# dakom/awsm-renderer

Hardware: AMD Instinct MI355X
Metric: frames/sec + shaded Mpix/s, 4K Sponza glTF, 1/2/4/8 MI355X (higher is better)
Workload: dtype f32; 1 GPU; Sponza-class procedural atrium (configs[3]): 262144 triangles, 25 materials, 69 textures, 3840x2160, geometry pass + opaque pass, single-sample, MipmapMode::None; triangles=262144, width=3840, height=2160, draws=92, frame_overlap=True, stream_handoff=device flags (k_handoff_signal / k_handoff_wait), camera=orbit, one turn per 240 frames, environment=uniform cubes (builder default), opaque_route=lean (k_shade_lean + k_shade_todo), library=awsm-renderer_amd/libawsm_hip.so

## Files before the change

### awsm-renderer_amd/csrc/awsm_hip.cpp

```cpp
#include <hip/hip_runtime.h>
#include <algorithm>
#include <cmath>
#include <cstdarg>
#include <cstdio>
#include <cstdlib>
#include <cstring>
#include <ctime>
#include <string>
#include <vector>

#include "ctx.hpp"
#include "launch.hpp"

using namespace awsm;

namespace {

constexpr int kLeanWgsPerCu = 0;

inline FrameBufs* pass_slots(AwsmHipCtx* c, PassKind kind) {
    FrameBufs* const sets[kPassKinds] = {c->fb, c->tr, c->hud, c->htr, c->shadow};
    return sets[kind];
}
inline FrameBufs& pass_bufs(AwsmHipCtx* c, PassKind kind) { return pass_slots(c, kind)[c->slot]; }
// ... 153 lines not shown
    return AWSM_OK;
}

uint32_t mip_levels_full(uint32_t w, uint32_t h) {
    uint32_t m = std::max(w, h), n = 0;
    while (m > 1u) { m >>= 1; n++; }
    return n + 1u;
}

}

namespace {

void shard(const AwsmHipCtx* c, uint32_t* y0, uint32_t* y1) {
    *y0 = c->y0; *y1 = c->y1;
    if (*y1 == 0 || *y1 > c->height) *y1 = c->height;
    if (*y0 > *y1) *y0 = *y1;
}

void log_dirty(AwsmHipCtx* c, AwsmBuf which, size_t lo, size_t hi) {
    if (c->geometry_cache) c->dirty_log.log((uint32_t)which, lo, hi, c->write_seq);
}

int sync_scene(AwsmHipCtx* c) {
    if (!c->scene_dirty) return AWSM_OK;
    c->write_seq++;
    { int rcb = scene_write_barrier(c, false); if (rcb) return rcb; }
    for (int i = 0; i < AWSM_BUF_COUNT; i++) c->scene.buf[i] = (const uint8_t*)c->bufs[i].ptr;
    c->scene.lut_rg16f = (const uint16_t*)c->lut.ptr;
    int rc = upload_small(c, c->scene_dev, &c->scene, sizeof(DevScene));
    if (rc) return rc;
    c->scene_dirty = false;
    c->scene_uploads++;
    return AWSM_OK;
}

void bind_pass(FrameDev& f, const FrameBufs& b) {
    f.bin_capacity = b.bin_capacity;
    f.draws = (const DrawDev*)b.draws_dev.ptr;
    f.clip = (float4*)b.clip.ptr; f.nrm = (float4*)b.nrm.ptr; f.tan = (float4*)b.tan.ptr;
    f.tri_info = (uint32_t*)b.tri_flags.ptr;
    f.tri_rec = (TriRec*)b.tri_rec.ptr;
    f.tile_count = (uint32_t*)b.tile_count.ptr; f.tile_offset = (uint32_t*)b.tile_offset.ptr;
    f.tile_cursor = (uint32_t*)b.tile_cursor.ptr; f.bin_list = (uint32_t*)b.bin_list.ptr;
    f.tile_order = (uint32_t*)b.tile_order.ptr;
    f.scan_tmp = (uint32_t*)b.scan_tmp.ptr;
    f.tile_split = (uint32_t*)b.tile_split.ptr; f.raster_scratch = (unsigned long long*)b.raster_scratch.ptr;
    f.raster_extra_cap = b.raster_extra_cap; f.raster_slot_cap = b.raster_slot_cap;
    f.big_list = (uint32_t*)b.big_list.ptr;
    f.counters = (uint32_t*)b.counters.ptr;
    f.vis = (unsigned long long*)b.vis.ptr;
}

struct FrameView { bool hud_keys, merged; };
inline FrameView world_view() { return {false, false}; }
inline FrameView frame_view(const AwsmHipCtx* c) { return {c->hud_geometry_done, c->hud_merged}; }

void fill_frame(AwsmHipCtx* c, FrameDev* f, FrameView view) {
    memset(f, 0, sizeof *f);
    const PassList& world = c->lists[kPassWorld];
    const PassList& hud = c->lists[kPassHud];
    uint32_t y0, y1;
    shard(c, &y0, &y1);
    f->width = c->width; f->height = c->height; f->y0 = y0; f->y1 = y1; f->sy0 = y0; f->sy1 = y1;
    if (c->msaa && (y0 > 0 || y1 < c->height)) {
        f->y0 = y0 > 0 ? y0 - 1 : 0; f->y1 = std::min(c->height, y1 + 1);
    }
    f->tiles_x = (c->width + kTile - 1) / kTile;
    f->band_n = 1; f->band_r = 0; f->out_compact = 0;
    f->tile_row0 = f->y0 >> kTileShift;
    f->tiles_y = (f->y1 > f->y0) ? ((f->y1 + kTile - 1) / kTile - f->tile_row0) : 0;
    if (c->band_n > 1) {
        const uint32_t rows_full = (c->height + kTile - 1) / kTile;
        f->band_n = c->band_n; f->band_r = c->band_r; f->out_compact = c->band_compact;
        f->tile_row0 = c->band_r;
        f->tiles_y = c->band_r < rows_full ? (rows_full - c->band_r + c->band_n - 1) / c->band_n : 0;
    }
    f->n_draws = (uint32_t)world.draws.size();
    f->total_tris = world.total_tris; f->total_verts = 3u * world.total_tris;
    bind_pass(*f, FB(c));
    f->draw_shade = (DrawShadeDev*)FB(c).draw_shade.ptr;
    f->tex_slots = (TexSlotDev*)FB(c).tex_slots.ptr;
    f->draw_mat = (DrawMatDev*)FB(c).draw_mat.ptr;
    const bool lean_ok = !(c->flags & AWSM_CFG_GENERAL_SHADE_ONLY) && (uint64_t)c->width * c->height * (c->msaa == 4 ? 32u : 8u) < (1ull << 32) && (c->msaa == 0 || (c->msaa_edge_bits[c->slot].ptr && c->msaa_cells[c->slot].ptr)) && FB(c).tri_shade.ptr && FB(c).draw_lean.ptr && c->shade_todo[c->slot].ptr && ((uint64_t)world.total_tris + (view.merged ? hud.total_tris : 0u)) * kTriRecBytes < (1ull << 32) &&
                         c->bufs[AWSM_BUF_ATTR_DATA].size < (1ull << 32) - 64;
    f->tri_shade = lean_ok ? (uint4*)FB(c).tri_shade.ptr : nullptr;
    f->attr_data_bytes = (uint32_t)std::min<size_t>(c->bufs[AWSM_BUF_ATTR_DATA].size, 0xFFFFFFFFu);
    f->draw_lean = lean_ok ? (LeanDrawDev*)FB(c).draw_lean.ptr : nullptr;
    f->shade_todo = (uint32_t*)c->shade_todo[c->slot].ptr;
    f->shade_todo_cap = f->shade_todo ? (uint32_t)(c->shade_todo[c->slot].size / 4 - 4 - 1024) : 0u;
    f->lean_next = f->shade_todo ? f->shade_todo + 4 + f->shade_todo_cap : nullptr;
    f->lean_grid = c->lean_grid;
#ifdef AWSM_STAMP
    {
        static unsigned long long* stamps = nullptr;
        if (!stamps && hipMalloc((void**)&stamps, 4ull * 16384 * 8 * 8) == hipSuccess) (void)hipMemset(stamps, 0, 4ull * 16384 * 8 * 8);
        f->stamps = stamps;
        static bool told = false;
        if (!told) { told = true; FILE* fp = fopen("/tmp/awsm_stamps_ptr", "w"); if (fp) { fprintf(fp, "%llu\n", (unsigned long long)(uintptr_t)stamps); fclose(fp); } }
    }
#endif
    f->poison = c->handoff_poison ? c->handoff_poison + c->slot : nullptr;
    f->host_bin_status = c->counters_host + 16 + 2 * c->slot;
    f->frame_serial = c->frame_serial;
    f->camera = (const uint8_t*)FB(c).camera.ptr;
    f->camera_snap = nullptr; f->camera_snap_words = 0;
    memcpy(f->pix2view, FB(c).pix2view, sizeof f->pix2view); memcpy(f->view_rot, FB(c).view_rot, sizeof f->view_rot); memcpy(f->cam_pos, FB(c).cam_pos, sizeof f->cam_pos);
    memcpy(f->ortho_view_dir, FB(c).ortho_view_dir, sizeof f->ortho_view_dir); f->cam_ortho = FB(c).cam_ortho;
    f->msaa = c->msaa;
    f->msaa_color0 = (float4*)c->msaa_color0[c->slot].ptr;
    f->msaa_edges = (uint32_t*)c->msaa_edges[c->slot].ptr;
    f->msaa_edge_bits = (lean_ok && c->msaa == 4) ? (unsigned long long*)c->msaa_edge_bits[c->slot].ptr : nullptr;
    f->msaa_cells = (uint2*)c->msaa_cells[c->slot].ptr;
    f->hud_vis = view.hud_keys ? (const unsigned long long*)c->hud[c->slot].vis.ptr : nullptr;
    f->hud_draws = (const DrawDev*)c->hud[c->slot].draws_dev.ptr; f->hud_tri_info = (const uint32_t*)c->hud[c->slot].tri_flags.ptr;
    if (view.hud_keys && view.merged) {
        f->n_draws = (uint32_t)c->hud_combined.size();
        f->total_tris = world.total_tris + hud.total_tris; f->total_verts = 3u * f->total_tris;
        f->vis = (unsigned long long*)c->merged_vis[c->slot].ptr;
        f->hud_draws = f->draws; f->hud_tri_info = f->tri_info;
    }
    f->hud_pass = 0;
    f->msaa_halo = (const unsigned long long*)c->msaa_halo;
    f->halo_bands = c->band_n > 1 ? ((c->height + kTile - 1) / kTile + c->band_n - 1) / c->band_n : 0u;
    f->out_rgba16f = (uint16_t*)(c->bound_out ? (uint8_t*)c->bound_out - (size_t)c->out_first_row * c->width * 8 : c->out16[c->slot].ptr);
    f->out_rgba32f = (float*)c->out32[c->slot].ptr;
    f->lights_pre = (float4*)c->lights_pre[c->slot].ptr;
    f->lights_cap = (uint32_t)(c->lights_pre[c->slot].size / 32);
}

void compose_pixel_to_view(AwsmHipCtx* c, FrameBufs& b) {
    float cam[128];
    memcpy(cam, c->camera_host, 512);
    const float* proj = cam + 16; const float* inv_proj = cam + 64; const float* inv_view = cam + 80;
    const double W = (double)c->width, H = (double)c->height;
    const double A[16] = {2.0 / W, 0, 0, 0,   0, -2.0 / H, 0, 0,   0, 0, 1, 0,   1.0 / W - 1.0, 1.0 - 1.0 / H, 0, 1};
    for (int col = 0; col < 4; col++) for (int row = 0; row < 4; row++) {
        double s = 0.0;
        for (int k = 0; k < 4; k++) s += (double)inv_proj[k * 4 + row] * A[col * 4 + k];
        b.pix2view[col * 4 + row] = (float)s;
    }
    for (int col = 0; col < 3; col++) for (int row = 0; row < 3; row++) b.view_rot[col * 3 + row] = inv_view[col * 4 + row];
    for (int i = 0; i < 3; i++) b.cam_pos[i] = cam[96 + i];
    b.cam_ortho = proj[15] > 0.9f ? 1u : 0u;
    const double vx = inv_view[8], vy = inv_view[9], vz = inv_view[10], l = std::sqrt(vx * vx + vy * vy + vz * vz);
    b.ortho_view_dir[0] = l > 0.0 ? (float)(vx / l) : 0.0f; b.ortho_view_dir[1] = l > 0.0 ? (float)(vy / l) : 0.0f; b.ortho_view_dir[2] = l > 0.0 ? (float)(vz / l) : 1.0f;
}

int record(AwsmHipCtx* c, int which, hipStream_t s = nullptr) {
    if (!c->stage_timers) { c->ev_valid[which] = false; return AWSM_OK; }
    HIPCHK(c, hipEventRecord(c->ev[which], s ? s : c->stream));
    c->ev_valid[which] = true;
    return AWSM_OK;
}

AwsmHipCtx::ResolveKey resolve_key(AwsmHipCtx* c, const FrameDev& f) {
    AwsmHipCtx::ResolveKey k;
    memset(&k, 0, sizeof k);
    k.write_seq = c->write_seq + (c->scene_dirty ? 1u : 0u); k.draws_version = FB(c).draws_version;
    k.ptrs[0] = f.draw_shade; k.ptrs[1] = f.draw_mat; k.ptrs[2] = f.tex_slots; k.ptrs[3] = f.draw_lean; k.ptrs[4] = f.lights_pre;
    k.n_draws = f.n_draws; k.mipmap = c->last_opaque.mipmap; k.has_opaque = c->last_opaque.has_opaque; k.lights_cap = f.lights_cap;
    return k;
}
bool resolve_stale(AwsmHipCtx* c, const FrameDev& f) {
    const AwsmHipCtx::ResolveKey k = resolve_key(c, f);
    return memcmp(&k, &c->resolved[c->slot], sizeof k) != 0;
}

void fill_geometry_cache(AwsmHipCtx* c, FrameDev* f, bool replay) {
    FrameBufs& b = FB(c);
    f->wcache = (float4*)b.wcache.ptr;
    f->cache_on = 0; f->prev_draws = nullptr; f->prev_n_draws = 0; f->n_dirty = 0; f->cache_serial = b.cache_serial;
    if (!c->geometry_cache || replay || !b.cache_valid || !b.wcache.ptr || b.cache_had_tri_shade != (f->tri_shade != nullptr)) return;
    std::vector<DirtyRange> r;
    if (!c->dirty_log.ranges_since(b.cache_seq, kMaxDirtyRanges, r)) return;
    for (size_t i = 0; i < r.size(); i++) { f->dirty[i][0] = r[i].buf; f->dirty[i][1] = r[i].lo; f->dirty[i][2] = r[i].hi; }
    f->n_dirty = (uint32_t)r.size();
    f->prev_draws = (const DrawDev*)(b.cached_is_prev ? b.draws_prev.ptr : b.draws_dev.ptr);
    f->prev_n_draws = b.cached_n_draws;
    f->cache_on = f->prev_draws ? 1u : 0u;
}


inline void enqueue_binning(const FrameDev& f, bool has_tris, hipStream_t s) {
    if (has_tris) { awsm_launch_bin_count(&f, s); awsm_launch_bin_big(&f, 0, s); }
    awsm_launch_bin_scan(&f, s);
    if (has_tris) { awsm_launch_bin_fill(&f, s); awsm_launch_bin_big(&f, 1, s); }
}
int clear_empty_pass(AwsmHipCtx* c, const FrameBufs& b, uint32_t n_tiles, hipStream_t s) {
    HIPCHK(c, hipMemsetAsync(b.counters.ptr, 0, kCtrWords * sizeof(uint32_t), s));
    HIPCHK(c, hipMemsetAsync((uint32_t*)b.counters.ptr + 12, 0, 2 * sizeof(uint32_t), s));
    if (n_tiles) HIPCHK(c, hipMemsetAsync(b.tile_count.ptr, 0, n_tiles * sizeof(uint32_t), s));
    return AWSM_OK;
}

int enqueue_geometry(AwsmHipCtx* c, bool replay = false) {
    HostTrace ht(c->frame_serial);
    const PassList& world = c->lists[kPassWorld];
    FrameDev f;
    fill_frame(c, &f, world_view());
    fill_geometry_cache(c, &f, replay);
    f.block_draw = FB(c).block_map_valid ? (const uint32_t*)FB(c).block_map.ptr : nullptr;
    f.cache_mark = (c->stage_timers && FB(c).cache_mark.size >= (size_t)world.n_blocks * 4) ? (uint32_t*)FB(c).cache_mark.ptr : nullptr;
    const uint32_t n_tiles = f.tiles_x * f.tiles_y;
    int rc = sync_scene(c);
    if (rc) return rc;
    ht.mark("geometry: sync_scene");
    if (c->overlap && c->shade_pending[c->slot]) { HIPCHK(c, wait_slot_free(c)); c->shade_pending[c->slot] = false; }
    if (c->bufs[AWSM_BUF_CAMERA].ptr && !replay) {
        const size_t cam_bytes = std::min<size_t>(512, c->bufs[AWSM_BUF_CAMERA].size);
        if (world.total_tris && n_tiles) { f.camera_snap = (uint32_t*)FB(c).camera.ptr; f.camera_snap_words = (uint32_t)(cam_bytes / 4); }
        else HIPCHK(c, hipMemcpyAsync(FB(c).camera.ptr, c->bufs[AWSM_BUF_CAMERA].ptr, cam_bytes, hipMemcpyDeviceToDevice, c->stream));
    }
    if (c->overlap) {
        c->uploads_recorded[c->slot] = false;
        if (resolve_stale(c, f)) { HIPCHK(c, hipEventRecord(c->ev_uploads[c->slot], c->stream)); c->uploads_recorded[c->slot] = true; }
        c->geom_write_seq[c->slot] = c->write_seq;
    }
    ht.mark("geometry: slot wait + upload event");
    const bool has_geometry = world.total_tris && n_tiles;
    if (!has_geometry && (rc = clear_empty_pass(c, FB(c), n_tiles, c->stream))) return rc;
    if (c->trace_dev) awsm_launch_handoff_signal(nullptr, 0u, trace_slot(c, 0), c->stream);
    if ((rc = record(c, EV_START))) return rc;
#ifdef AWSM_DEBUG_SWITCHES
    static const int knockout_env = getenv("AWSM_DEBUG_KNOCKOUT") ? atoi(getenv("AWSM_DEBUG_KNOCKOUT")) : 0;
    const int knockout = c->frame_serial > 8 ? knockout_env : 0;
#else
    const int knockout = 0;
#endif
    if (has_geometry && !(knockout & 1)) awsm_launch_transform(c->scene_dev, &f, world.n_blocks, c->stream);
    if ((rc = record(c, EV_TRANSFORM))) return rc;
    ht.mark("geometry: transform launch");
    if (n_tiles && !(knockout & 2)) enqueue_binning(f, world.total_tris != 0, c->stream);
    if ((rc = record(c, EV_BIN))) return rc;
    ht.mark("geometry: bin launches");
    if (n_tiles && !(knockout & 4)) awsm_launch_raster(&f, c->stream);
    if ((rc = record(c, EV_RASTER))) return rc;
    ht.mark("geometry: raster launch");
    HIPCHK(c, hipGetLastError());
    {
        FrameBufs& b = FB(c);
        b.cache_valid = has_geometry && !(knockout & 1) && b.wcache.ptr != nullptr;
        b.cached_n_draws = (uint32_t)world.draws.size(); b.cached_is_prev = false;
// ... 402 lines not shown
    if (hipGetDeviceProperties(&prop, c->device) != hipSuccess) return bail(AWSM_ERR_DEVICE);
    if (strncmp(prop.gcnArchName, "gfx950", 6) != 0) {
        fprintf(stderr, "awsm_hip: device %d is %s; this library carries gfx950 code objects only\n", c->device, prop.gcnArchName);
        return bail(AWSM_ERR_NO_DEVICE);
    }
    if (cfg->stream) { c->stream = (hipStream_t)cfg->stream; c->own_stream = false; }
    else { if (hipStreamCreateWithFlags(&c->stream, hipStreamNonBlocking) != hipSuccess) return bail(AWSM_ERR_DEVICE); c->own_stream = true; }
    for (int i = 0; i < EV_COUNT; i++) if (hipEventCreate(&c->ev[i]) != hipSuccess) return bail(AWSM_ERR_DEVICE);
    if (hipMalloc((void**)&c->scene_dev, sizeof(DevScene)) != hipSuccess) return bail(AWSM_ERR_OUT_OF_MEMORY);
    c->overlap = (cfg->flags & AWSM_CFG_OVERLAP_FRAMES) != 0;
    { const char* e = getenv("AWSM_GEOMETRY_CACHE"); c->geometry_cache = !(e && e[0] == '0'); }
    {
        const char* e = getenv("AWSM_LEAN_WGS_PER_CU");
        const int per_cu = e ? atoi(e) : (c->overlap ? kLeanWgsPerCu : 0);
        c->lean_grid = per_cu > 0 ? (uint32_t)(per_cu * prop.multiProcessorCount) & ~7u : 0u;
    }
    for (int s = 0; s < n_slots(c); s++) {
        for (PassKind k : {kPassWorld, kPassTransparent, kPassHudTransparent, kPassHud}) {
            DevBuf& ctr = pass_slots(c, k)[s].counters;
            if (hipMalloc(&ctr.ptr, 16 * sizeof(uint32_t)) != hipSuccess || (k == kPassWorld && hipMemset(ctr.ptr, 0, 16 * sizeof(uint32_t)) != hipSuccess)) return bail(AWSM_ERR_OUT_OF_MEMORY);
            ctr.size = 16 * sizeof(uint32_t);
        }
        if (hipMalloc(&c->fb[s].camera.ptr, 512) != hipSuccess || hipMemset(c->fb[s].camera.ptr, 0, 512) != hipSuccess) return bail(AWSM_ERR_OUT_OF_MEMORY);
        c->fb[s].camera.size = 512;
    }

    if (c->overlap) {
        for (int s = 0; s < kSlots; s++) {
#ifdef AWSM_DEBUG_SWITCHES
            if (const char* m = getenv("AWSM_SHADE_CU_MASK")) {
                std::vector<uint32_t> words;
                for (const char* p = m; *p; ) { char* end = nullptr; words.push_back((uint32_t)strtoul(p, &end, 16)); p = (*end == ',') ? end + 1 : end; if (end == p && *p) break; }
                if (words.empty() || hipExtStreamCreateWithCUMask(&c->shade_streams[s], (uint32_t)words.size(), words.data()) != hipSuccess) return bail(AWSM_ERR_DEVICE);
            } else
#endif
            if (hipStreamCreateWithFlags(&c->shade_streams[s], hipStreamNonBlocking) != hipSuccess) return bail(AWSM_ERR_DEVICE);
            const unsigned ev_flags = hipEventDisableTiming | hipEventReleaseToDevice;
            if (hipEventCreateWithFlags(&c->ev_geom_done[s], ev_flags) != hipSuccess || hipEventCreateWithFlags(&c->ev_shade_done[s], ev_flags) != hipSuccess ||
                hipEventCreateWithFlags(&c->ev_uploads[s], ev_flags) != hipSuccess) return bail(AWSM_ERR_DEVICE);
            if (s == 0 && hipEventCreateWithFlags(&c->ev_flush, hipEventDisableTiming) != hipSuccess) return bail(AWSM_ERR_DEVICE);
        }
    }
    if (hipHostMalloc((void**)&c->counters_host, (16 + 2 * kSlots + 1) * sizeof(uint32_t), hipHostMallocDefault) != hipSuccess) return bail(AWSM_ERR_OUT_OF_MEMORY);
    memset(c->counters_host, 0, (16 + 2 * kSlots + 1) * sizeof(uint32_t));
    if (c->overlap) {
        const char* e = getenv("AWSM_DEVICE_HANDOFF");
        c->handoff = !(e && e[0] == '0');
        { int khz = 0; if (hipDeviceGetAttribute(&khz, hipDeviceAttributeWallClockRate, c->device) == hipSuccess && khz > 0) c->clock_khz = (uint32_t)khz; }
        double budget_ms = 4000.0;
        if (const char* p = getenv("AWSM_HANDOFF_TIMEOUT_MS")) { const double v = atof(p); if (v > 0.0) budget_ms = v; }
        c->handoff_budget_ticks = (unsigned long long)(budget_ms * (double)c->clock_khz) + 1ull;
        if (hipMalloc((void**)&c->handoff_flags, 3 * kSlots * sizeof(uint32_t)) != hipSuccess || hipMalloc((void**)&c->handoff_poison, kSlots * sizeof(uint32_t)) != hipSuccess) return bail(AWSM_ERR_OUT_OF_MEMORY);
        if (hipMemset(c->handoff_flags, 0, 3 * kSlots * sizeof(uint32_t)) != hipSuccess || hipMemset(c->handoff_poison, 0xFF, kSlots * sizeof(uint32_t)) != hipSuccess ||
            hipDeviceSynchronize() != hipSuccess) return bail(AWSM_ERR_DEVICE);
        if (const char* d = getenv("AWSM_TEST_HANDOFF_DROP")) c->handoff_test_drop = (uint32_t)atoi(d);
        for (int k = 0; c->handoff && k < 2 * kSlots; k++) {
            hipStream_t ss = c->shade_streams[k % kSlots], waiter = k < kSlots ? ss : c->stream, setter = k < kSlots ? c->stream : ss;
            const uint32_t serial = ++c->geom_sig[0];
            awsm_launch_handoff_wait(c->handoff_flags, serial, 10ull * c->clock_khz , handoff_timeouts(c), 0u, nullptr, 0u, waiter);
            awsm_launch_handoff_signal(c->handoff_flags, serial, nullptr, setter);
            if (hipStreamSynchronize(waiter) != hipSuccess || hipStreamSynchronize(setter) != hipSuccess) return bail(AWSM_ERR_DEVICE);
            if (*(volatile uint32_t*)handoff_timeouts(c) != 0u) { c->handoff = false; c->handoff_timeouts_seen = *(volatile uint32_t*)handoff_timeouts(c); }
        }
    }
    memset(&c->scene, 0, sizeof c->scene);
    c->scene.skybox_rgba[3] = 1.0f;
    for (int i = 0; i < 3; i++) { c->scene.prefiltered_rgb[i] = 1.0f; c->scene.irradiance_rgb[i] = 1.0f; }
    *out = c;
    return AWSM_OK;
}

int awsm_hip_destroy(AwsmHipCtx* c) {
    if (!c) return AWSM_ERR_INVALID_ARGUMENT;
    (void)hipSetDevice(c->device);
    if (c->stream) (void)hipStreamSynchronize(c->stream);
    (void)sync_shade_streams(c);
    auto fr = [](DevBuf& b) { if (b.ptr) (void)hipFree(b.ptr); b.ptr = nullptr; b.size = 0; };
    for (auto& b : c->bufs) fr(b);
    for (auto& b : c->tex) fr(b);
    for (auto& b : c->tex_kinds) fr(b);
    for (auto& b : c->merged_vis) fr(b);
    fr(c->pose_records);
    fr(c->env_stage); fr(c->env_tables); fr(c->env_rows); fr(c->env_filter_tab); if (c->ev_env_copy) (void)hipEventDestroy(c->ev_env_copy);
    fr(c->lut); for (auto& b : c->cube_tex) fr(b); for (auto& b : c->cube_bordered) fr(b); fr(c->digest); for (auto& b : c->shade_todo) fr(b); for (int sl = 0; sl < kSlots; sl++) { fr(c->msaa_color0[sl]); fr(c->msaa_edges[sl]); fr(c->msaa_edge_bits[sl]); fr(c->msaa_cells[sl]); } fr(c->mip_kinds); for (auto& b : c->out16) fr(b); for (auto& b : c->out32) fr(b); fr(c->comp16); fr(c->comp32); fr(c->grid_layer); for (auto& b : c->lights_pre) fr(b);
    for (auto& b : c->ssao_layers) fr(b);
    for (auto& b : c->taa_img) fr(b); fr(c->taa_layers);
    for (auto& b : c->sel_tables) fr(b);
    fr(c->sel_layers);
    for (auto& b : c->shadow_layers) fr(b); for (auto& b : c->shadow_cam) fr(b); for (DevScene* sc : c->shadow_scene) if (sc) (void)hipFree(sc);
    for (auto& b : c->display8) fr(b); fr(c->effects16); fr(c->bloom_a); fr(c->bloom_b); fr(c->dof_lc); fr(c->dof_blur);
    for (int k = 0; k < kPassKinds * kSlots; k++) {
        FrameBufs& b = pass_slots(c, (PassKind)(k / kSlots))[k % kSlots];
        fr(b.vis); fr(b.wpos); fr(b.frag_rec); fr(b.frag_color); fr(b.frag_first); fr(b.tex_slots); fr(b.draw_mat); fr(b.clip); fr(b.nrm); fr(b.tan); fr(b.tri_rec); fr(b.tri_flags); fr(b.tri_shade); fr(b.draw_lean); fr(b.draws_dev); fr(b.draw_shade); fr(b.tile_count); fr(b.tile_offset);
        fr(b.wcache); fr(b.draws_prev); fr(b.cache_mark); fr(b.block_map); fr(b.tile_cursor); fr(b.tile_order); fr(b.scan_tmp); fr(b.tile_split); fr(b.raster_scratch); fr(b.bin_list); fr(b.big_list); fr(b.counters); fr(b.camera);
    }
    for (hipStream_t st : c->shade_streams) if (st) (void)hipStreamDestroy(st);
    for (int i = 0; i < kSlots; i++) { if (c->ev_geom_done[i]) (void)hipEventDestroy(c->ev_geom_done[i]); if (c->ev_shade_done[i]) (void)hipEventDestroy(c->ev_shade_done[i]); if (c->ev_uploads[i]) (void)hipEventDestroy(c->ev_uploads[i]); }
    if (c->ev_flush) (void)hipEventDestroy(c->ev_flush);
    if (c->scene_dev) (void)hipFree(c->scene_dev);
    if (c->stage) (void)hipHostFree(c->stage);
    if (c->counters_host) (void)hipHostFree(c->counters_host);
    if (c->handoff_flags) (void)hipFree(c->handoff_flags);
    if (c->handoff_poison) (void)hipFree(c->handoff_poison);
    if (c->trace_dev) (void)hipFree(c->trace_dev);
    for (int i = 0; i < EV_COUNT; i++) if (c->ev[i]) (void)hipEventDestroy(c->ev[i]);
    if (c->own_stream && c->stream) (void)hipStreamDestroy(c->stream);
    delete c;
    return AWSM_OK;
}

int awsm_hip_device_info(AwsmHipCtx* c, char* name_out, size_t name_cap, uint32_t* cu_count, uint64_t* hbm_bytes) {
    if (!c) return AWSM_ERR_INVALID_ARGUMENT;
    hipDeviceProp_t prop;
    HIPCHK(c, hipGetDeviceProperties(&prop, c->device));
    if (name_out && name_cap) snprintf(name_out, name_cap, "%s (%s)", prop.name, prop.gcnArchName);
    if (cu_count) *cu_count = (uint32_t)prop.multiProcessorCount;
    if (hbm_bytes) *hbm_bytes = (uint64_t)prop.totalGlobalMem;
    return AWSM_OK;
}

int awsm_hip_buffer_create(AwsmHipCtx* c, AwsmBuf which, size_t bytes) {
    if (!c || (int)which < 0 || which >= AWSM_BUF_COUNT) return fail(c, AWSM_ERR_INVALID_ARGUMENT, "buffer_create: bad buffer id %d", (int)which);
    HIPCHK(c, hipSetDevice(c->device));
    { int rcb = scene_write_barrier(c); if (rcb) return rcb; }
    log_dirty(c, which, 0, ~size_t(0));
    if (bytes && c->bufs[which].ptr && c->bufs[which].size == bytes) {
        if (which == AWSM_BUF_CAMERA) memset(c->camera_host, 0, sizeof c->camera_host);
        HIPCHK(c, hipMemsetAsync(c->bufs[which].ptr, 0, bytes + 16, c->stream));
        return AWSM_OK;
    }
    int rc = dev_realloc(c, c->bufs[which], bytes ? bytes + 16 : 0, true);
    if (rc) return rc;
    if (bytes) c->bufs[which].size = bytes;
    if (which == AWSM_BUF_CAMERA) memset(c->camera_host, 0, sizeof c->camera_host);
    if (which == AWSM_BUF_LIGHTS) for (int sl = 0; sl < n_slots(c); sl++) if ((rc = dev_realloc(c, c->lights_pre[sl], std::max<size_t>(bytes / 64, 1) * 32, true))) return rc;
    c->scene_dirty = true;
    return AWSM_OK;
}

int awsm_hip_buffer_write(AwsmHipCtx* c, AwsmBuf which, size_t dst_off, const void* src, size_t len) {
    if (!c || (int)which < 0 || which >= AWSM_BUF_COUNT || (!src && len)) return fail(c, AWSM_ERR_INVALID_ARGUMENT, "buffer_write: bad argument");
    if ((dst_off & 3) || (len & 3)) return fail(c, AWSM_ERR_INVALID_ARGUMENT, "buffer_write: offset %zu / size %zu not 4-byte aligned", dst_off, len);
    DevBuf& b = c->bufs[which];
    if (!b.ptr) return fail(c, AWSM_ERR_NOT_READY, "buffer_write: buffer %d was never created", (int)which);
    if (dst_off > b.size || len > b.size - dst_off) return fail(c, AWSM_ERR_OUT_OF_RANGE, "buffer_write: [%zu,+%zu) outside buffer %d of %zu bytes", dst_off, len, (int)which, b.size);
    if (len == 0) return AWSM_OK;
    HIPCHK(c, hipSetDevice(c->device));
    if (which != AWSM_BUF_CAMERA) { int rcb = scene_write_barrier(c); if (rcb) return rcb; log_dirty(c, which, dst_off, dst_off + len); }
    else { if (dst_off < 512) memcpy(c->camera_host + dst_off, src, std::min<size_t>(len, 512 - dst_off)); c->camera_written_since_snapshot = true; }
    uint8_t* dst = (uint8_t*)b.ptr + dst_off;
    if (len <= (1u << 20)) return upload_small(c, dst, src, len);
    HIPCHK(c, hipMemcpyAsync(dst, src, len, hipMemcpyHostToDevice, c->stream));
    HIPCHK(c, hipStreamSynchronize(c->stream));
    return AWSM_OK;
}

int awsm_hip_skin_pose_records_write(AwsmHipCtx* c, uint32_t first, uint32_t n, const AwsmSkinPoseRecord* records) {
    if (!c || (!records && n)) return fail(c, AWSM_ERR_INVALID_ARGUMENT, "skin_pose_records_write: bad argument");
    static_assert(sizeof(AwsmSkinPoseRecord) == 72, "k_skin_pose reads 72-byte records");
    std::vector<AwsmSkinPoseRecord>& host = c->pose_records_host;
    if (first > host.size() || n > 0x03000000u - first) return fail(c, AWSM_ERR_OUT_OF_RANGE, "skin_pose_records_write: [%u,+%u) with %zu records resident", first, n, host.size());
    if (n == 0) return AWSM_OK;
    for (uint32_t i = 0; i < n; i++)
        if ((records[i].transform_offset & 3u) || (records[i].matrix_offset & 3u)) return fail(c, AWSM_ERR_INVALID_ARGUMENT, "skin_pose_records_write: record %u has an offset that is not a multiple of 4", first + i);
    HIPCHK(c, hipSetDevice(c->device));
    { int rcb = scene_write_barrier(c, false); if (rcb) return rcb; }
    std::vector<AwsmSkinPoseRecord> next(host.begin(), host.end());
// ... 6 lines not shown
        if (rc) { host.clear(); return rc; }
        lo = 0; count = next.size();
    }
    constexpr size_t kChunk = 8192;
    for (size_t at = lo; at < lo + count; at += kChunk) {
        const size_t m = std::min(kChunk, lo + count - at);
        int rc = upload_small(c, (uint8_t*)c->pose_records.ptr + at * sizeof(AwsmSkinPoseRecord), next.data() + at, m * sizeof(AwsmSkinPoseRecord));
        if (rc) { host.clear(); return rc; }
    }
    host.swap(next);
    return AWSM_OK;
}

int awsm_hip_skin_pose(AwsmHipCtx* c, const uint32_t* ids, uint32_t n) {
    if (!c || (!ids && n)) return fail(c, AWSM_ERR_INVALID_ARGUMENT, "skin_pose: bad argument");
    if (n == 0) return AWSM_OK;
    const DevBuf& tb = c->bufs[AWSM_BUF_TRANSFORMS];
    const DevBuf& mb = c->bufs[AWSM_BUF_SKIN_MATRICES];
    if (!tb.ptr || !mb.ptr) return fail(c, AWSM_ERR_NOT_READY, "skin_pose: the transforms or the skin matrices buffer was never created");
    const std::vector<AwsmSkinPoseRecord>& host = c->pose_records_host;
    std::vector<uint32_t> offs(n);
    for (uint32_t i = 0; i < n; i++) {
        if (ids[i] >= host.size()) return fail(c, AWSM_ERR_OUT_OF_RANGE, "skin_pose: record id %u (list entry %u) with %zu records resident", ids[i], i, host.size());
        const AwsmSkinPoseRecord& r = host[ids[i]];
        if (tb.size < 64 || r.transform_offset > tb.size - 64) return fail(c, AWSM_ERR_OUT_OF_RANGE, "skin_pose: record %u reads [%u,+64) of a transforms buffer of %zu bytes", ids[i], r.transform_offset, tb.size);
        if (mb.size < 64 || r.matrix_offset > mb.size - 64) return fail(c, AWSM_ERR_OUT_OF_RANGE, "skin_pose: record %u writes [%u,+64) of a skin matrices buffer of %zu bytes", ids[i], r.matrix_offset, mb.size);
        offs[i] = r.matrix_offset;
    }
    HIPCHK(c, hipSetDevice(c->device));
    { int rcb = scene_write_barrier(c); if (rcb) return rcb; }
    std::sort(offs.begin(), offs.end());
    for (size_t i = 0; i < offs.size();) {
        size_t j = i + 1;
        while (j < offs.size() && offs[j] <= offs[j - 1] + 64u) j++;
        log_dirty(c, AWSM_BUF_SKIN_MATRICES, offs[i], (size_t)offs[j - 1] + 64);
        i = j;
    }
    constexpr uint32_t kChunk = 65536;
    for (uint32_t at = 0; at < n; at += kChunk) {
        const uint32_t m = std::min(kChunk, n - at);
        uint8_t* st;
        int rc = stage_alloc(c, (size_t)m * 4, &st);
        if (rc) return rc;
        memcpy(st, ids + at, (size_t)m * 4);
        awsm_launch_skin_pose(c->pose_records.ptr, (const uint32_t*)st, m, tb.ptr, mb.ptr, c->stream);
        HIPCHK(c, hipGetLastError());
    }
    return AWSM_OK;
}

int awsm_hip_buffer_read(AwsmHipCtx* c, AwsmBuf which, size_t offset, void* dst, size_t len) {
    if (!c || (int)which < 0 || which >= AWSM_BUF_COUNT || (!dst && len)) return fail(c, AWSM_ERR_INVALID_ARGUMENT, "buffer_read: bad argument");
    const DevBuf& b = c->bufs[which];
    if (!b.ptr) return fail(c, AWSM_ERR_NOT_READY, "buffer_read: buffer %d was never created", (int)which);
    if (offset > b.size || len > b.size - offset) return fail(c, AWSM_ERR_OUT_OF_RANGE, "buffer_read: [%zu,+%zu) outside buffer %d of %zu bytes", offset, len, (int)which, b.size);
    if (len == 0) return AWSM_OK;
    HIPCHK(c, hipSetDevice(c->device));
    HIPCHK(c, hipStreamSynchronize(c->stream));
    HIPCHK(c, hipMemcpy(dst, (const uint8_t*)b.ptr + offset, len, hipMemcpyDeviceToHost));
    return AWSM_OK;
}

int awsm_hip_resize(AwsmHipCtx* c, uint32_t width, uint32_t height, uint32_t msaa) {
    if (!c || width == 0 || height == 0 || width > 16384 || height > 16384) return fail(c, AWSM_ERR_INVALID_ARGUMENT, "resize: bad size %ux%u", width, height);
    if (msaa == 1) msaa = 0;
    if (msaa != 0 && msaa != 4) return fail(c, AWSM_ERR_UNSUPPORTED, "resize: MSAA x%u (the reference supports None or 4, anti_alias.rs:28-38)", msaa);
    HIPCHK(c, hipSetDevice(c->device));
    const size_t px = (size_t)width * height, samples = msaa == 4 ? 4 : 1;
    int rc;
    if ((rc = sync_all(c))) return rc;
    for (int s = 0; s < n_slots(c); s++) {
        if ((rc = dev_realloc(c, c->fb[s].vis, px * samples * 8, false))) return rc;
        HIPCHK(c, hipMemsetAsync(c->fb[s].vis.ptr, 0xFF, px * samples * 8, c->stream));
    }
    if (msaa == 4) for (int sl = 0; sl < n_slots(c); sl++) {
        const size_t blocks = (size_t)((width + 15) / 16) * ((height + 15) / 16);
        if ((rc = dev_realloc(c, c->msaa_edge_bits[sl], blocks * 4 * 16, true))) return rc;
        if ((rc = dev_realloc(c, c->msaa_cells[sl], px * 8, false))) return rc;
        if ((rc = dev_realloc(c, c->msaa_color0[sl], px * 16, false))) return rc;
        if ((rc = dev_realloc(c, c->msaa_edges[sl], blocks * 260, false))) return rc;
    }
    c->msaa = msaa;
    for (int sl = 0; sl < n_slots(c); sl++) if ((rc = dev_realloc(c, c->shade_todo[sl], ((size_t)((width + 15) / 16) * ((height + 15) / 16) * 4 + 4 + 1024) * 4, true))) return rc;
    for (int sl = 0; sl < n_slots(c); sl++) {
        if ((rc = dev_realloc(c, c->out16[sl], px * 8, true))) return rc;
        if ((c->flags & AWSM_CFG_PARITY_TAP) && (rc = dev_realloc(c, c->out32[sl], px * 16, true))) return rc;
    }
    c->width = width; c->height = height;
    c->y0 = c->y1 = 0;
    c->band_n = 1; c->band_r = 0; c->band_compact = 0;
    c->geometry_done = c->opaque_done = c->transparent_done = c->hud_transparent_done = c->post_done = false;
    c->last_display = nullptr;
    c->taa_have = false; c->taa_serial = 0; c->taa_resolved = false;
    return AWSM_OK;
}

int awsm_hip_set_shard_bands(AwsmHipCtx* c, uint32_t n, uint32_t r, uint32_t compact_output) {
    if (!c) return AWSM_ERR_INVALID_ARGUMENT;
    if (c->width == 0) return fail(c, AWSM_ERR_NOT_READY, "set_shard_bands before resize");
    if (n == 0 || r >= n) return fail(c, AWSM_ERR_INVALID_ARGUMENT, "set_shard_bands: need r < n (got n=%u r=%u)", n, r);
    { int rcs = sync_all(c); if (rcs) return rcs; }
    c->y0 = c->y1 = 0;
    c->band_n = n; c->band_r = n > 1 ? r : 0; c->band_compact = (n > 1 && compact_output) ? 1u : 0u;
    return AWSM_OK;
}

uint32_t awsm_hip_msaa_halo_bands(AwsmHipCtx* c) {
    return (c && c->band_n > 1 && c->height) ? ((c->height + kTile - 1) / kTile + c->band_n - 1) / c->band_n : 0u;
}

int awsm_hip_msaa_halo_export(AwsmHipCtx* c, void* dst, size_t bytes) {
    if (!c || !dst) return AWSM_ERR_INVALID_ARGUMENT;
    if (c->msaa != 4 || c->band_n <= 1) return fail(c, AWSM_ERR_INVALID_ARGUMENT, "msaa_halo_export: only for MSAA x4 with band sharding");
    if (!c->geometry_done) return fail(c, AWSM_ERR_NOT_READY, "msaa_halo_export before geometry_pass");
    const uint32_t bands = awsm_hip_msaa_halo_bands(c);
    if (bytes < (size_t)bands * 2 * c->width * 8) return fail(c, AWSM_ERR_INVALID_ARGUMENT, "msaa_halo_export: %zu bytes, %zu needed (%u bands x 2 rows x %u keys)", bytes, (size_t)bands * 2 * c->width * 8, bands, c->width);
    HIPCHK(c, hipSetDevice(c->device));
    FrameDev f;
    fill_frame(c, &f, frame_view(c));
    awsm_launch_msaa_halo_export(&f, (unsigned long long*)dst, bands, c->stream);
    HIPCHK(c, hipGetLastError());
    return AWSM_OK;
}

int awsm_hip_msaa_halo_bind(AwsmHipCtx* c, const void* gathered, size_t bytes) {
    if (!c) return AWSM_ERR_INVALID_ARGUMENT;
    if (gathered && bytes == 0) return fail(c, AWSM_ERR_INVALID_ARGUMENT, "msaa_halo_bind: zero-sized array");
    c->msaa_halo = gathered; c->msaa_halo_bytes = bytes;
    return AWSM_OK;
}

int awsm_hip_set_shard_rows(AwsmHipCtx* c, uint32_t y0, uint32_t y1) {
    if (!c) return AWSM_ERR_INVALID_ARGUMENT;
    if (c->width == 0) return fail(c, AWSM_ERR_NOT_READY, "set_shard_rows before resize");
    { int rcs = sync_all(c); if (rcs) return rcs; }
    c->band_n = 1; c->band_r = 0; c->band_compact = 0;
    if (y0 == 0 && y1 == 0) { c->y0 = c->y1 = 0; return AWSM_OK; }
    if (y0 >= y1 || y1 > c->height) return fail(c, AWSM_ERR_INVALID_ARGUMENT, "set_shard_rows: need y0 < y1 <= height (got %u,%u)", y0, y1);

    c->y0 = y0; c->y1 = y1;
    return AWSM_OK;
}

int awsm_hip_geometry_pass(AwsmHipCtx* c, const AwsmDraw* draws, uint32_t n) {
    if (!c || (!draws && n)) return AWSM_ERR_INVALID_ARGUMENT;
    if (c->width == 0) return fail(c, AWSM_ERR_NOT_READY, "geometry_pass before resize");
    static const AwsmBuf need[] = {AWSM_BUF_TRANSFORMS, AWSM_BUF_CAMERA, AWSM_BUF_GEOM_META, AWSM_BUF_VIS_GEOM_DATA};
    if (n) for (AwsmBuf b : need) if (!c->bufs[b].ptr) return fail(c, AWSM_ERR_NOT_READY, "geometry_pass: buffer %d missing", (int)b);
    HIPCHK(c, hipSetDevice(c->device));

    HostTrace ht(c->frame_serial + 1u);
    std::vector<DrawDev> new_draws;
    uint64_t tris = 0, blocks = 0;
    int rc = build_draw_list(c, "geometry_pass", draws, n, AWSM_BUF_VIS_GEOM_DATA, 168u, new_draws, &tris, &blocks);
    if (rc) return rc;
    ht.mark("geometry_pass: draw list");
    if ((rc = handoff_check(c))) return rc;
    c->hud_geometry_done = false; c->hud_merged = false;
    c->frame_serial++;
    if (c->overlap) {
        c->slot = (c->slot + 1) % kSlots;
        if (c->shade_pending[c->slot]) {
            if (hipEventQuery(c->ev_shade_done[c->slot]) != hipSuccess) HIPCHK(c, wait_slot_free(c));
            c->shade_pending[c->slot] = false;
        }
    }
// ... 953 lines not shown
```

### awsm-renderer_amd/csrc/ctx.hpp

```cpp
#pragma once
#include <hip/hip_runtime.h>
#include <stddef.h>
#include <stdint.h>
#include <string>
#include <vector>

#include "frame_params.hpp"
#include "dirty_log.hpp"

namespace awsm {

#ifndef AWSM_SLOTS
#define AWSM_SLOTS 2
#endif
constexpr int kSlots = AWSM_SLOTS;
struct DevBuf {
    void* ptr = nullptr;
    size_t size = 0;
};

enum { EV_START = 0, EV_TRANSFORM, EV_BIN, EV_RASTER, EV_SHADE_BEGIN, EV_SHADE_LEAN, EV_SHADE, EV_FWD_BEGIN, EV_FWD, EV_COUNT };

enum PassKind : uint8_t { kPassWorld = 0, kPassTransparent, kPassHud, kPassHudTransparent, kPassShadow };
constexpr int kPassKinds = 5;
// ... 12 lines not shown
    DevBuf tri_shade, draw_lean;
    DevBuf clip, nrm, tan, tri_rec, tri_flags, draws_dev, draw_shade, tile_count, tile_offset, tile_cursor, tile_order, bin_list, big_list, counters, vis;
    DevBuf camera;
    DevBuf scan_tmp;
    DevBuf tile_split, raster_scratch;
    uint32_t raster_extra_cap = 0, raster_slot_cap = 0;
    uint32_t bin_capacity = 0;
    float pix2view[16] = {}, view_rot[9] = {}, cam_pos[3] = {}, ortho_view_dir[3] = {};
    uint32_t cam_ortho = 0;
    size_t tri_cap = 0, draw_cap = 0;
    uint32_t sized_w = 0, sized_h = 0;
    std::vector<DrawDev> draws_uploaded;
    void* draws_uploaded_ptr = nullptr;
    bool draws_uploaded_valid = false;
    uint64_t draws_version = 0;
    std::vector<DrawDev> tail_uploaded;
    void* tail_uploaded_ptr = nullptr;
    size_t tail_uploaded_at = 0;
    bool tail_uploaded_valid = false;
    DevBuf wcache, draws_prev;
    DevBuf block_map;
    bool block_map_valid = false;
    DevBuf cache_mark;
    uint32_t cached_n_draws = 0;
    bool cache_valid = false;
    bool cached_is_prev = false;
    bool cache_had_tri_shade = false;
    uint64_t cache_seq = 0;
    uint32_t cache_serial = 0;
    PassKind kind = kPassWorld;
    uint8_t slot = 0;
};

}

using namespace awsm;

struct AwsmHipCtx {
    int device = 0;
    uint32_t flags = 0;
    hipStream_t stream = nullptr;
    bool own_stream = false;
    bool stage_timers = true;
    std::string last_error;

    DevBuf bufs[AWSM_BUF_COUNT];
    bool camera_written_since_snapshot = false;
    uint8_t camera_host[512] = {};
    DevScene scene{};
    DevScene* scene_dev = nullptr;
    bool scene_dirty = true;
    DevBuf tex[kMaxTexArrays];
    DevBuf lut;
    DevBuf cube_tex[3], cube_bordered[3];
    DevBuf env_stage, env_tables, env_rows, env_filter_tab;
    hipEvent_t ev_env_copy = nullptr;
    DevBuf tex_kinds[kMaxTexArrays];
    uint32_t tex_srgb[64] = {};
    bool tex_srgb_made = false;

    DevBuf pose_records;
    std::vector<AwsmSkinPoseRecord> pose_records_host;

    uint32_t width = 0, height = 0;
    uint32_t y0 = 0, y1 = 0;
    uint32_t band_n = 1, band_r = 0, band_compact = 0;
    uint32_t msaa = 0;
    DevBuf mip_kinds;
    DevBuf msaa_color0[kSlots], msaa_edges[kSlots];
    DevBuf msaa_edge_bits[kSlots];
    DevBuf msaa_cells[kSlots];
    DevBuf out16[kSlots], out32[kSlots];
    DevBuf digest;
    uint32_t lean_grid = 0;
    DevBuf shade_todo[kSlots];
    void* bound_out = nullptr;
    size_t bound_out_bytes = 0;
    const uint8_t* slot_out_lo[kSlots] = {}; const uint8_t* slot_out_hi[kSlots] = {};

    bool overlap = false;
    hipStream_t shade_streams[kSlots] = {};
    bool shade_recorded[kSlots] = {};
    bool uploads_recorded[kSlots] = {};
    struct ResolveKey { uint64_t write_seq, draws_version; const void* ptrs[5]; uint32_t n_draws, mipmap, has_opaque, lights_cap; } resolved[kSlots] = {};
    hipEvent_t ev_geom_done[kSlots] = {}, ev_shade_done[kSlots] = {}, ev_uploads[kSlots] = {} ;
    hipEvent_t ev_flush = nullptr;
    uint64_t write_seq = 0, geom_write_seq[kSlots] = {};
    DirtyLog dirty_log;
    bool geometry_cache = true;
    uint32_t cache_blocks_last = 0;
    bool shade_pending[kSlots] = {};
    bool handoff = false;
    uint32_t* handoff_flags = nullptr;
    uint32_t geom_sig[kSlots] = {}, shade_sig[kSlots] = {}, lean_sig[kSlots] = {};
    bool lean_flagged[kSlots] = {};
    unsigned long long handoff_budget_ticks = 400000000ull;
    uint32_t clock_khz = 100000;
    uint32_t* handoff_poison = nullptr;
    uint32_t handoff_timeouts_seen = 0;
    uint32_t handoff_dropped_frames = 0;
    bool handoff_error_pending = false;
    uint32_t handoff_test_drop = 0;
    FrameBufs fb[kSlots];
    FrameBufs tr[kSlots];
    FrameBufs hud[kSlots];
    bool hud_geometry_done = false;
    bool hud_merged = false;
    DevBuf merged_vis[kSlots];
    std::vector<DrawDev> hud_combined;
    bool transparent_done = false, hud_transparent_done = false;
    FrameBufs htr[kSlots];
    struct GridState { bool on = false; float p[20] = {}; } grid, grid_pass[kSlots];
    DevBuf grid_layer;
    struct SelectionState {
        bool on = false;
        uint32_t flags = 0, radius = 0;
        float outline_color[4] = {}, box_color[4] = {}, half_width = 0, hidden_alpha = 0, depth_epsilon = 0;
        std::vector<uint32_t> keys;
        std::vector<float> boxes;
    } sel, sel_pass[kSlots];
    DevBuf sel_tables[kSlots], sel_layers;
    DevBuf comp16, comp32;
    DevBuf display8[kSlots], effects16, bloom_a, bloom_b, dof_lc, dof_blur;
    void* bound_display = nullptr;
    size_t bound_display_bytes = 0;
    void* last_display = nullptr;
    bool post_done = false;
    AwsmPostParams post_params{};
    DevBuf lights_pre[kSlots];
    void* bound_comp = nullptr;
    size_t bound_comp_bytes = 0;
    const void* msaa_halo = nullptr;
    size_t msaa_halo_bytes = 0;
    const void* opaque_src = nullptr;
    size_t opaque_src_bytes = 0;
    int slot = 0;
    PassList lists[kPassKinds];
    std::vector<AwsmDraw> draws_api;
    bool geometry_done = false, opaque_done = false;
    AwsmOpaqueParams last_opaque{};
    uint32_t overflow_retries = 0;
    bool has_opaque_for_stats() const { return !opaque_done || last_opaque.has_opaque != 0; }

    uint8_t* stage = nullptr;
    size_t stage_cap = 0, stage_head = 0;
    uint32_t* counters_host = nullptr;
    uint32_t frame_serial = 0, status_seen[kSlots] = {};
    uint32_t dropped_frames = 0;
    uint32_t out_first_row = 0;
    bool out_rows_mode = false;

    hipEvent_t ev[EV_COUNT] = {};
    bool ev_valid[EV_COUNT] = {};

    unsigned long long* trace_dev = nullptr;
    uint32_t trace_cap = 0;

    struct SsaoState { bool on = false; float p[4] = {}; } ssao, ssao_pass[kSlots];
    DevBuf ssao_layers[kSlots];
    size_t ssao_px[kSlots] = {};

    FrameBufs shadow[kSlots];
    DevScene* shadow_scene[kSlots] = {};
    uint64_t shadow_scene_seq[kSlots] = {}, scene_uploads = 0;
    DevBuf shadow_cam[kSlots];
    bool shadow_done = false;
    struct ShadowState { bool on = false; AwsmShadow p{}; float light_view_proj[16] = {}; } shadow_pass[kSlots];
    DevBuf shadow_layers[kSlots];
    size_t shadow_px[kSlots] = {};

    struct TaaState {
        bool on = false;
        float feedback = 0.1f;
        uint32_t flags = 0;
        float jitter[2] = {};
        float reproject[16] = {1, 0, 0, 0, 0, 1, 0, 0, 0, 0, 1, 0, 0, 0, 0, 1};
    } taa, taa_pass;
    DevBuf taa_img[2], taa_layers;
    int taa_cur = 0;
    bool taa_have = false;
    bool taa_frame_hist = false;
    uint32_t taa_serial = 0;
    bool taa_resolved = false;
    TaaArgs taa_args{};
};

#define HIPCHK(c, call)                                                                            \
    do {                                                                                           \
        hipError_t e_ = (call);                                                                    \
        if (e_ != hipSuccess)                                                                      \
            return fail((c), e_ == hipErrorOutOfMemory ? AWSM_ERR_OUT_OF_MEMORY : AWSM_ERR_DEVICE, \
                        "%s failed: %s (%s:%d)", #call, hipGetErrorString(e_), __FILE__, __LINE__); \
    } while (0)

#define AWSM_HIDDEN __attribute__((visibility("hidden")))

namespace awsm {

AWSM_HIDDEN int fail(AwsmHipCtx* c, int code, const char* fmt, ...);
AWSM_HIDDEN hipError_t sync_shade_streams(AwsmHipCtx* c);
AWSM_HIDDEN int dev_realloc(AwsmHipCtx* c, DevBuf& b, size_t bytes, bool zero);
AWSM_HIDDEN int dev_reserve(AwsmHipCtx* c, DevBuf& b, size_t bytes);
AWSM_HIDDEN int stage_alloc(AwsmHipCtx* c, size_t len, uint8_t** out);
AWSM_HIDDEN int upload_small(AwsmHipCtx* c, void* dst, const void* src, size_t len);
AWSM_HIDDEN int scene_write_barrier(AwsmHipCtx* c, bool is_write = true);
AWSM_HIDDEN int sync_all(AwsmHipCtx* c);
AWSM_HIDDEN uint32_t mip_levels_full(uint32_t w, uint32_t h);

}
```

### awsm-renderer_amd/csrc/frame_params.hpp

```cpp
#pragma once
#include <hip/hip_runtime.h>
#include <stdint.h>
#include "../../include/awsm_hip.h"

namespace awsm {

constexpr int kTile = 32;
constexpr int kTileShift = 5;
constexpr int kMaxTexArrays = 64;
constexpr int kMaxSamplers = 32;

constexpr uint32_t kDrawInstanced = 0x80u;

struct DrawDev {
    uint32_t geom_meta_off;
    uint32_t vis_data_off;
    uint32_t tri_count;
    uint32_t flags;
    uint32_t first_tri;
    uint32_t first_block;
    uint32_t inst_off;
    uint32_t pad1;
};

struct DrawShadeDev {
    uint32_t first_tri;
    uint32_t material_word;
    uint32_t attr_indices_word;
    uint32_t attr_data_word;
    uint32_t stride_words;
    uint32_t uv_sets_index;
    uint32_t flags;
    uint32_t color_sets;
};

struct TexSlotDev {
    const uint32_t* base;
    uint32_t width, height;
    uint32_t flags;
    float tt[6];
    uint32_t layer_levels;
    const uint32_t* level_off;
    const uint32_t* array_base;
};
static_assert(sizeof(TexSlotDev) == 64, "TexSlotDev must be 64 bytes");
constexpr int kCoreTextures = 5;

struct DrawMatDev {
    float base_color[4];
    float metallic, roughness, normal_scale, occlusion_strength;
    float emissive[3];
    float ior;
    uint32_t shader_alpha;
    uint32_t debug_bitmask;
    uint32_t ext_mask;
    float alpha_cutoff;
};
static_assert(sizeof(DrawMatDev) == 64, "DrawMatDev must be 64 bytes");

struct LeanDrawDev {
    uint32_t flags;
    float metallic, roughness, normal_scale;
    float base_color[3]; float occlusion_strength;
    float emissive[3];
    float normal_bias;
    uint32_t tex[kCoreTextures][2];
    float occlusion_bias;
    uint32_t pad1;
    uint32_t gtex[kCoreTextures][4];
    float tt[6];
    uint32_t pad2[2];
};
static_assert(sizeof(LeanDrawDev) == 208, "LeanDrawDev must be 208 bytes");

constexpr int kMaxMipLevels = 16;
struct TexArrayDev {
    const uint8_t* texels;
    uint32_t width, height, layers;
    uint32_t mips;
    uint32_t level_off[kMaxMipLevels];
};

struct CubeDev {
    const uint2* texels;
    uint32_t size, mips;
    uint32_t level_off[kMaxMipLevels];
    const uint2* bordered;
    uint32_t b_level_off[kMaxMipLevels];
};
enum { kCubeSkybox = 0, kCubePrefiltered = 1, kCubeIrradiance = 2 };

struct DevScene {
    const uint8_t* buf[AWSM_BUF_COUNT];
    TexArrayDev tex[kMaxTexArrays];
    AwsmSampler samplers[kMaxSamplers];
    uint32_t n_tex, n_samplers;
    float skybox_rgba[4];
    float prefiltered_rgb[4];
    float irradiance_rgb[4];
    const uint16_t* lut_rg16f;
    uint32_t lut_w, lut_h;
    CubeDev cube[3];
};

struct TriRec;
constexpr size_t kTriRecBytes = 80;
constexpr uint32_t kMaxDirtyRanges = 12;

enum CounterWord : uint32_t { kCtrBinned = 0, kCtrEntries, kCtrOverflow, kCtrCovered, kCtrBig, kCtrFragments, kCtrFragOverflow, kCtrExtraItems, kCtrWords };

struct FrameDev {
    uint32_t width, height;
    uint32_t y0, y1;
    uint32_t sy0, sy1;
    uint32_t tiles_x, tiles_y;
    uint32_t tile_row0;
    uint32_t band_n, band_r;
    uint32_t out_compact;
    uint32_t n_draws;
    uint32_t total_tris;
    uint32_t total_verts;
    uint32_t rank0, block0;
    uint32_t bin_capacity;
    uint32_t has_opaque;
    uint32_t mipmap;
    uint32_t aniso;
    uint32_t msaa;
    const uint8_t* camera;
    float pix2view[16];
    float view_rot[9];
    float cam_pos[3];
    float ortho_view_dir[3];
    uint32_t cam_ortho;
    const DrawDev* draws;
    DrawShadeDev* draw_shade;
    TexSlotDev* tex_slots;
    DrawMatDev* draw_mat;
    float4* lights_pre;
    uint32_t lights_cap;
    float4* clip;
    float4* nrm;
    float4* tan;
    float4* wpos;
    const uint32_t* block_draw;
    float4* wcache;
    const DrawDev* prev_draws;
    uint32_t prev_n_draws;
    uint32_t cache_on;
    uint32_t cache_serial;
    uint32_t* cache_mark;
    uint32_t n_dirty;
    uint32_t dirty[12][3];
    TriRec* tri_rec;
    uint32_t* tri_info;
    uint4* tri_shade;
    uint32_t attr_data_bytes;
    LeanDrawDev* draw_lean;
    uint32_t* shade_todo;
    uint32_t shade_todo_cap;
    uint32_t* lean_done_flag;
    uint32_t lean_done_serial;
    uint32_t* camera_snap;
    uint32_t camera_snap_words;
    uint32_t* lean_next;
    uint32_t lean_grid;
    uint32_t* tile_count;
    uint32_t* tile_offset;
    uint32_t* tile_cursor;
    uint32_t* scan_tmp;
    uint32_t* tile_order;
    uint32_t* tile_split;
    unsigned long long* raster_scratch;
    uint32_t raster_extra_cap, raster_slot_cap;
    uint32_t* bin_list;
    uint32_t* big_list;
#ifdef AWSM_STAMP
    unsigned long long* stamps;
#endif
    const uint32_t* poison;
    uint32_t* host_bin_status;
    uint32_t frame_serial;
    uint32_t* counters;
    unsigned long long* vis;
    uint16_t* out_rgba16f;
    float* out_rgba32f;
    float4* msaa_color0;
    uint32_t* msaa_edges;
    unsigned long long* msaa_edge_bits;
    uint2* msaa_cells;
    const unsigned long long* hud_vis;
    const DrawDev* hud_draws;
    const uint32_t* hud_tri_info;
    uint32_t hud_pass;
    const unsigned long long* msaa_halo;
    uint32_t halo_bands;
    const uint16_t* opaque_rgba16f;
    uint4* frag_rec;
    float4* frag_color;
    uint32_t* frag_first;
    uint32_t frag_cap;
};

struct PostArgs {
    uint32_t width, height;
    const uint2* src;
    const unsigned long long* vis;
    const uint32_t* frag_first;
    const uint4* frag_rec;
    uint32_t frag_cap;
    const TriRec* tri_rec;
    const float* camera;
    float2* dof_lc;
    float4* dof_blur;
    const uint2* stage_in;
    uint2* stage_out;
    uint2* effects;
    uint32_t* display;
    uint32_t tonemap;
    uint32_t dof;
    const uint32_t* poison;
    uint32_t frame_serial;
};
// ... 61 lines not shown
```

### awsm-renderer_amd/csrc/kernels_shade.hip

```cpp
#include <type_traits>
#include "shade_gbuffer.hpp"
#include "shade_samplers.hpp"
#include "cube_seam.hpp"
#include "editor_grid.hpp"
#include "launch.hpp"

#ifndef AWSM_LEAN_WAVES
#define AWSM_LEAN_WAVES 6
#endif

namespace awsm {

#pragma clang fp contract(fast)

AWSM_DI f4 half4(uint2 h) { return {f16_bits_to_f32((unsigned short)(h.x & 0xFFFFu)), f16_bits_to_f32((unsigned short)(h.x >> 16)), f16_bits_to_f32((unsigned short)(h.y & 0xFFFFu)), f16_bits_to_f32((unsigned short)(h.y >> 16))}; }
AWSM_DI f4 cube_texel(const CubeDev& c, uint32_t level_base, int N, uint32_t face, int i, int j) { return half4(cube_texel_raw(c, level_base, N, face, i, j)); }
__global__ __launch_bounds__(256) void k_cube_border(CubeDev c, uint2* __restrict__ out, uint32_t total) {
    const uint32_t idx = blockIdx.x * 256u + threadIdx.x;
    if (idx >= total) return;
    uint32_t level = 0u;
    while (level + 1u < c.mips && idx >= c.b_level_off[level + 1u]) level++;
    const int N = (int)max(c.size >> level, 1u), P = N + 2;
    const uint32_t r = idx - c.b_level_off[level], face = r / (uint32_t)(P * P), q = r % (uint32_t)(P * P);
    out[idx] = cube_texel_raw(c, c.level_off[level], N, face, (int)(q % (uint32_t)P) - 1, (int)(q / (uint32_t)P) - 1);
// ... 192 lines not shown
        const float4 pre0 = lights_pre[i * 2], pre1 = lights_pre[i * 2 + 1];
        const uint32_t kind = (uint32_t)pre0.w;
        f3 light_dir = {pre0.x, pre0.y, pre0.z}, radiance = {pre1.x, pre1.y, pre1.z};
        if (kind == 2u || kind == 3u) {
            const float4 pos_range = lights[i * 4 + 0];
            const f3 stl = mk3(pos_range.x, pos_range.y, pos_range.z) - world_position;
            const float d2 = fm::fdot(stl, stl);
            const float inv_d = d2 > 0.0f ? fm::rsq(d2) : 0.0f;
            const float dist = d2 * inv_d;
            float att;
            if (pos_range.w == 0.0f) att = fm::rcp(fmaxf(dist * dist, 0.01f));
            else { const float fo = 1.0f - fm::fdiv(dist * dist, pos_range.w * pos_range.w); att = fm::fdiv(saturate(fo * fo), dist * dist + 1.0f); }
            const f3 to_light = stl * inv_d;
            if (kind == 3u) {
                const float4 dir_inner = lights[i * 4 + 1], kind_outer = lights[i * 4 + 3];
                const float cos_l = fm::fdot(to_light, -light_dir);
                const float sm = saturate(fm::fdiv(cos_l - kind_outer.y, dir_inner.w - kind_outer.y));
                att = att * (sm * sm);
            }
            light_dir = to_light;
            radiance = radiance * att;
        } else if (kind != 1u) { light_dir = {0.0f, 0.0f, 0.0f}; radiance = {0.0f, 0.0f, 0.0f}; }
        color = color + brdf_direct(mc, sf, light_dir, radiance);
    }
    return color;
}

AWSM_DI void store_pixel(const FrameDev& f, size_t p, f4 c) {
    ushort4 h = make_ushort4(f16_bits(c.x), f16_bits(c.y), f16_bits(c.z), f16_bits(c.w));
    __builtin_nontemporal_store(*reinterpret_cast<unsigned long long*>(&h), reinterpret_cast<unsigned long long*>(f.out_rgba16f) + p);
    if (f.out_rgba32f) reinterpret_cast<float4*>(f.out_rgba32f)[p] = make_float4(c.x, c.y, c.z, c.w);
}

AWSM_DI TexSlotDev resolve_tex_slot(const DevScene* __restrict__ sc, const uint32_t* __restrict__ M, const uint32_t (&words)[kCoreTextures], int k, bool unlit) {
    TexSlotDev s;
    s.base = nullptr; s.width = 0u; s.height = 0u; s.flags = 0u; s.layer_levels = 0u; s.level_off = nullptr; s.array_base = nullptr;
    for (int j = 0; j < 6; j++) s.tt[j] = 0.0f;
    if (!(unlit && k >= 2)) {
        const TexInfo t = tex_load(M, words[k]);
        if (t.exists) {
            s.flags = 1u | (t.uv_set_index << 24);
            const float* tt = reinterpret_cast<const float*>(sc->buf[AWSM_BUF_TEXTURE_TRANSFORMS] + (size_t)t.uv_transform_index * 32u);
            for (int j = 0; j < 6; j++) s.tt[j] = tt[j];
            bool ok = t.array_index < sc->n_tex && t.sampler_index < sc->n_samplers;
            if (ok) {
                const TexArrayDev& arr = sc->tex[t.array_index];
                const AwsmSampler& smp = sc->samplers[t.sampler_index];
                ok = arr.texels != nullptr && arr.width != 0u && arr.height != 0u && arr.layers != 0u;
                if (ok) {
                    const uint32_t layer = min(t.layer_index, arr.layers - 1u);
                    s.base = reinterpret_cast<const uint32_t*>(arr.texels) + (size_t)layer * arr.width * arr.height;
                    s.width = arr.width; s.height = arr.height;
                    const bool common = smp.address_mode_u == 1u && smp.address_mode_v == 1u && (arr.width & (arr.width - 1u)) == 0u && (arr.height & (arr.height - 1u)) == 0u;
                    if (common && smp.mag_filter != 0u) s.flags |= 2u;
                    if (common) s.flags |= 8u;
                    s.flags |= (smp.mag_filter != 0u ? 16u : 0u) | (smp.min_filter != 0u ? 32u : 0u) | (smp.mipmap_filter != 0u ? 64u : 0u);
                    s.flags |= ((smp.address_mode_u & 3u) << 13) | ((smp.address_mode_v & 3u) << 21);
                    const uint32_t an = (smp.mag_filter != 0u && smp.min_filter != 0u && smp.mipmap_filter != 0u) ? min(max(smp.max_anisotropy, 1u), 16u) : 1u;
                    s.layer_levels = (layer & 0xFFFFu) | (an << 16) | (max(arr.mips, 1u) << 24);
                    s.level_off = &sc->tex[t.array_index].level_off[0];
                    s.array_base = reinterpret_cast<const uint32_t*>(arr.texels);
                }
            }
            if (!ok) s.flags |= 4u;
        }
    }
    return s;
}

__global__ __launch_bounds__(256) void k_resolve_draws(const DevScene* __restrict__ sc, FrameDev f) {
    const uint32_t d = blockIdx.x * 256u + threadIdx.x;
    if (f.lights_pre && sc->buf[AWSM_BUF_LIGHTS_INFO] && sc->buf[AWSM_BUF_LIGHTS]) {
        const uint32_t n_lights = min(*reinterpret_cast<const uint32_t*>(sc->buf[AWSM_BUF_LIGHTS_INFO]), f.lights_cap);
        const float4* lights = reinterpret_cast<const float4*>(sc->buf[AWSM_BUF_LIGHTS]);
        for (uint32_t i = d; i < n_lights; i += gridDim.x * 256u) {
            const float4 dir_inner = lights[i * 4 + 1], color_intensity = lights[i * 4 + 2], kind_outer = lights[i * 4 + 3];
            const uint32_t kind = (uint32_t)kind_outer.x;
            f3 v = {dir_inner.x, dir_inner.y, dir_inner.z};
            if (kind == 1u) v = fm::fsafe_normalize(-v);
            else v = fm::fnormalize(v);
            f.lights_pre[i * 2] = make_float4(v.x, v.y, v.z, kind_outer.x);
            f.lights_pre[i * 2 + 1] = make_float4(color_intensity.x * color_intensity.w, color_intensity.y * color_intensity.w, color_intensity.z * color_intensity.w, 0.0f);
        }
    }
    if (d == 0u && f.shade_todo) f.shade_todo[0] = 0u;
    if (d < 64u && f.lean_next) f.lean_next[d * 16u] = 0u;
    const uint32_t draw = d >> 3, role = d & 7u;
    if (draw >= f.n_draws || role > 6u) return;
    const DrawDev dr = f.draws[draw];
    const uint32_t material_meta_offset = *reinterpret_cast<const uint32_t*>(sc->buf[AWSM_BUF_GEOM_META] + dr.geom_meta_off + 36);
    const uint32_t* mm = reinterpret_cast<const uint32_t*>(sc->buf[AWSM_BUF_MATERIAL_META] + (size_t)(material_meta_offset / 256u) * 256u);
    const uint32_t* M = reinterpret_cast<const uint32_t*>(sc->buf[AWSM_BUF_MATERIALS]);
    const uint32_t material_word = mm[6] / 4u, b = material_word + 1u;
    const uint32_t shader_id = M[material_word];
    const bool unlit = shader_id == 2u;
    const uint32_t words[kCoreTextures] = {b + 2u, b + 11u, b + 18u, b + 24u, b + 30u};
    if (role == 6u) {
        if (!f.draw_lean) return;
        LeanDrawDev L;
        L.flags = 0u; L.normal_bias = 1.0f; L.occlusion_bias = 1.0f; L.pad1 = 0u; L.pad2[0] = 0u; L.pad2[1] = 0u;
        L.tt[0] = 1.0f; L.tt[1] = 0.0f; L.tt[2] = 0.0f; L.tt[3] = 1.0f; L.tt[4] = 0.0f; L.tt[5] = 0.0f;
        bool have_tt = false;
        L.metallic = 0.0f; L.roughness = 0.0f; L.normal_scale = 1.0f; L.occlusion_strength = 1.0f;
        for (int j = 0; j < 3; j++) { L.base_color[j] = 0.0f; L.emissive[j] = 0.0f; }
        for (int k = 0; k < kCoreTextures; k++) { L.tex[k][0] = 0u; L.tex[k][1] = 0u; for (int j = 0; j < 4; j++) L.gtex[k][j] = 0u; }
        bool lean_grad = true, lean_aniso = true;
        uint32_t aniso = 0u;
        bool lean = shader_id == 1u && (mm[16] & 1u) == 0u && M[b + 38] == 0u;
        if (lean) {
            const uint32_t fi = b + 39u;
            for (int j = 0; j < 12; j++) if (M[fi + j] != 0u) lean = false;
        }
        if (lean) {
            uint32_t exists = 0u;
            for (int k = 0; k < kCoreTextures && lean; k++) {
                const TexSlotDev s = resolve_tex_slot(sc, M, words, k, false);
                if (!(s.flags & 1u)) continue;
                const unsigned long long addr = (unsigned long long)s.base;
                bool same_tt = true;
                for (int j = 0; j < 6; j++) { if (!have_tt) L.tt[j] = s.tt[j]; else if (__float_as_uint(L.tt[j]) != __float_as_uint(s.tt[j])) same_tt = false; }
                have_tt = true;
                if ((s.flags & 6u) != 2u || (s.flags >> 24) != 0u || !same_tt || s.width > 32768u || s.height > 32768u || (addr >> 48) != 0ull || (addr & 3ull) != 0ull) { lean = false; break; }
                exists |= 1u << k;
                L.tex[k][0] = (uint32_t)addr;
                L.tex[k][1] = (uint32_t)(addr >> 32) | ((uint32_t)(31 - __clz((int)s.width)) << 16) | ((uint32_t)(31 - __clz((int)s.height)) << 20);
                {
                    const TexInfo ti = tex_load(M, words[k]);
                    const TexArrayDev& arr = sc->tex[ti.array_index];
                    const unsigned long long abase = (unsigned long long)s.array_base;
                    const uint32_t levels = s.layer_levels >> 24, layer = s.layer_levels & 0xFFFFu, lw = (uint32_t)(31 - __clz((int)s.width));
                    unsigned long long chain_texels = 0ull;
                    for (uint32_t l = 0; l < levels; l++) chain_texels += (unsigned long long)arr.layers * max(arr.width >> l, 1u) * max(arr.height >> l, 1u);
                    const bool ok = s.width == s.height && (s.flags & (32u | 64u)) == (32u | 64u) && levels >= 1u && levels <= 15u && levels <= lw + 1u && arr.layers < 4096u &&
                                    chain_texels * 4ull < 0xFFFFFFF0ull && (abase >> 48) == 0ull && (abase & 3ull) == 0ull;
                    if (!ok) lean_grad = false;
                    const uint32_t an = max((s.layer_levels >> 16) & 31u, 1u);
                    if (aniso != 0u && an != aniso) lean_aniso = false;
                    aniso = an;
                    L.gtex[k][0] = (uint32_t)abase; L.gtex[k][1] = (uint32_t)(abase >> 32) | (levels << 16) | (lw << 24);
                    L.gtex[k][2] = layer; L.gtex[k][3] = arr.layers;
                }
            }
            if (lean) {
                const bool identity = L.tt[0] == 1.0f && L.tt[1] == 0.0f && L.tt[2] == 0.0f && L.tt[3] == 1.0f && L.tt[4] == 0.0f && L.tt[5] == 0.0f;
                L.flags = 1u | (lean_grad ? 2u : 0u) | (lean_grad && lean_aniso ? 4u : 0u) | (identity ? 0u : 8u) | (exists << 8);
                L.pad1 = f.aniso ? max(aniso, 1u) : 1u;
                const float k255 = 1.0f / 255.0f;
                const float s_base = (exists & 1u) ? k255 : 1.0f, s_mr = (exists & 2u) ? k255 : 1.0f, s_em = (exists & 16u) ? k255 : 1.0f;
                L.metallic = mf(M, b + 16) * s_mr; L.roughness = mf(M, b + 17) * s_mr;
                const float nscale = mf(M, b + 23), ostrength = mf(M, b + 29);
                L.normal_scale = (nscale * 2.0f) * k255; L.normal_bias = nscale;
                L.occlusion_strength = (exists & 8u) ? ostrength * k255 : 0.0f; L.occlusion_bias = (exists & 8u) ? 1.0f - ostrength : 1.0f;
                const float strength = M[b + 39u + 1u] != 0u ? mf(M, b + M[b + 39u + 1u]) : 1.0f;
                for (int j = 0; j < 3; j++) { L.base_color[j] = mf(M, b + 7 + j) * s_base; L.emissive[j] = (mf(M, b + 35 + j) * strength) * s_em; }
            }
        }
        if (!(L.flags & 1u)) for (int k = 0; k < kCoreTextures; k++) { L.tex[k][0] = 0u; L.tex[k][1] = 0u; for (int j = 0; j < 4; j++) L.gtex[k][j] = 0u; }
        f.draw_lean[draw] = L;
        return;
    }
    if (role == 5u) {
        DrawShadeDev o;
        o.first_tri = dr.first_tri;
        o.material_word = material_word;
        o.attr_indices_word = mm[9] / 4u; o.attr_data_word = mm[10] / 4u; o.stride_words = mm[11] / 4u;
        o.uv_sets_index = mm[12];
// ... 648 lines not shown
    const uint32_t nblk = bx_n * by_n;
    const uint32_t xcd = wg & 7u, k = wg >> 3;
    const uint32_t rows_x = (by_n + 7u - xcd) >> 3;
    if (k >= rows_x * bx_n) return false;
    b.blk = ((k / bx_n) * 8u + xcd) * bx_n + (k % bx_n);
    if (b.blk >= nblk) return false;
    b.brow = b.blk / bx_n;
    b.x0 = (int)((b.blk % bx_n) << 4);
    b.y0 = f.band_n > 1u ? (int)(((f.tile_row0 + (b.brow >> 1) * f.band_n) << kTileShift) + ((b.brow & 1u) << 4)) : (int)f.sy0 + (int)(b.brow << 4);
    return true;
}
AWSM_DI void shade_block_at(const FrameDev& f, ShadeBlock& b, uint32_t brow, uint32_t bcol) {
    const uint32_t bx_n = (f.width + 15u) >> 4;
    b.blk = brow * bx_n + bcol;
    b.brow = brow;
    b.x0 = (int)(bcol << 4);
    b.y0 = f.band_n > 1u ? (int)(((f.tile_row0 + (brow >> 1) * f.band_n) << kTileShift) + ((brow & 1u) << 4)) : (int)f.sy0 + (int)(brow << 4);
}

template <int GRAD>
AWSM_DI void shade_pixel(const DevScene* __restrict__ sc, const FrameDev& f, const ShadeBlock& b, uint32_t tid) {
    const int cx = b.x0 + (int)(tid & 15u), cy = b.y0 + (int)(tid >> 4);
    if (cx >= (int)f.width || cy >= (int)f.sy1) return;
    const size_t pv = (size_t)cy * f.width + (size_t)cx;
    const size_t p = f.out_compact ? (size_t)(((b.brow >> 1) << kTileShift) + (uint32_t)(cy & (kTile - 1))) * f.width + (size_t)cx : pv;
    const unsigned long long key = f.vis[pv];
    if (f.hud_vis && f.has_opaque && f.hud_vis[pv] != ~0ull) { store_pixel(f, p, f4{0.0f, 0.0f, 0.0f, 0.0f}); return; }
    if (!f.has_opaque || key == ~0ull) { store_pixel(f, p, skybox_color(sc, f, cx, cy)); return; }
    const uint32_t rank = key_rank(key);
    const GBufferTexel g = reconstruct_gbuffer<(GRAD != 0)>(f, rank, cx, cy);
    const SurfaceOut o = shade_surface<GRAD>(sc, f, rank, cx, cy, key_depth(key), g, true);
    store_pixel(f, p, o.kind == 2u ? f4{0.0f, 0.0f, 0.0f, 0.0f} : o.color);
}
template <int GRAD>
__global__ __launch_bounds__(256) __attribute__((amdgpu_waves_per_eu(GRAD ? 4 : 5))) void k_shade(const DevScene* __restrict__ sc, FrameDev f) {
    ShadeBlock b;
    if (frame_poisoned(f) || !shade_block(f, b)) return;
    shade_pixel<GRAD>(sc, f, b, threadIdx.x);
}
template <int GRAD>
AWSM_DI void shade_pixel_msaa0(const DevScene* __restrict__ sc, const FrameDev& f, const ShadeBlock& b, uint32_t tid) {
    const int cx = b.x0 + (int)(tid & 15u), cy = b.y0 + (int)(tid >> 4);
    if (cx >= (int)f.width || cy >= (int)f.sy1) return;
    const size_t pv = (size_t)cy * f.width + (size_t)cx;
    const size_t p = f.out_compact ? (size_t)(((b.brow >> 1) << kTileShift) + (uint32_t)(cy & (kTile - 1))) * f.width + (size_t)cx : pv;
    const unsigned long long* masks = f.msaa_edge_bits + (size_t)(b.blk * 4u + (tid >> 6)) * 2u;
    const bool want_c0 = (((masks[0] | masks[1]) >> (tid & 63u)) & 1ull) != 0ull;
    const unsigned long long key = f.vis[pv * 4];
    if (key == ~0ull) return;
    const uint32_t rank = key_rank(key);
    const GBufferTexel g = reconstruct_gbuffer<(GRAD != 0)>(f, rank, cx, cy);
    const SurfaceOut o = shade_surface<GRAD>(sc, f, rank, cx, cy, key_depth(key), g, true);
    store_pixel(f, p, o.kind == 2u ? f4{0.0f, 0.0f, 0.0f, 0.0f} : o.color);
    if (want_c0) f.msaa_color0[pv] = o.kind != 0u ? make_float4(0.0f, 0.0f, 0.0f, __uint_as_float(0xFFFFFFFFu)) : make_float4(o.color.x, o.color.y, o.color.z, o.color.w);
}
constexpr uint32_t kTodoBlocks = 1024;
template <int GRAD, bool MSAA>
__global__ __launch_bounds__(256) __attribute__((amdgpu_waves_per_eu(4))) void k_shade_todo(const DevScene* __restrict__ sc, FrameDev f) {
    if (f.lean_done_flag && blockIdx.x == 0u && threadIdx.x == 0u) __hip_atomic_store(f.lean_done_flag, f.lean_done_serial, __ATOMIC_RELAXED, __HIP_MEMORY_SCOPE_AGENT);
    if (frame_poisoned(f)) return;
    const uint32_t n = min(f.shade_todo[0], f.shade_todo_cap);
    const uint32_t lane = threadIdx.x & 63u;
    const uint32_t wave = (uint32_t)__builtin_amdgcn_readfirstlane((int)(threadIdx.x >> 6));
    for (uint32_t i = blockIdx.x * 4u + wave; i < n; i += kTodoBlocks * 4u) {
        const uint32_t e = (uint32_t)__builtin_amdgcn_readfirstlane((int)f.shade_todo[4u + i]);
        ShadeBlock b;
        if (!shade_block(f, b, e >> 2)) continue;
        if (MSAA) shade_pixel_msaa0<GRAD>(sc, f, b, ((e & 3u) << 6) | lane);
        else shade_pixel<GRAD>(sc, f, b, ((e & 3u) << 6) | lane);
    }
}

#define AWSM_AS1 __attribute__((address_space(1)))
#define AWSM_AS4 __attribute__((address_space(4)))
typedef uint32_t u32x2 __attribute__((ext_vector_type(2)));
typedef uint32_t u32x2a4 __attribute__((ext_vector_type(2), aligned(4)));
typedef uint32_t u32x4 __attribute__((ext_vector_type(4)));
typedef float f32x2a4 __attribute__((ext_vector_type(2), aligned(4)));
typedef float f32x4 __attribute__((ext_vector_type(4)));
typedef double f64x2 __attribute__((ext_vector_type(2)));
template <typename T> AWSM_DI T gload(const void* base, uint32_t byte_off) { return *(const AWSM_AS1 T*)((const AWSM_AS1 char*)base + byte_off); }
template <typename T> AWSM_DI T gload64(unsigned long long base, uint32_t byte_off) { return *(const AWSM_AS1 T*)((const AWSM_AS1 char*)base + byte_off); }
template <typename T> AWSM_DI T cload(const void* base, uint32_t byte_off) { return *(const AWSM_AS4 T*)((const AWSM_AS4 char*)base + byte_off); }
AWSM_DI float4 as_float4(f32x4 v) { return make_float4(v.x, v.y, v.z, v.w); }
AWSM_DI m4 cload_m4(const void* base, uint32_t byte_off) {
    m4 m;
#pragma unroll
    for (int i = 0; i < 4; i++) { const f32x4 v = cload<f32x4>(base, byte_off + 16u * i); m.c[i] = {v.x, v.y, v.z, v.w}; }
    return m;
}

namespace lean {
struct Tap { uint32_t t00, t10, t01, t11; float fx, fy; };
struct Tex { unsigned long long base; uint32_t lw, lh; };
AWSM_DI Tex decode(uint32_t lo, uint32_t hi) { return {((unsigned long long)(hi & 0xFFFFu) << 32) | lo, (hi >> 16) & 15u, (hi >> 20) & 15u}; }
AWSM_DI void fetch(const Tex& x, float u, float v, Tap& t) {
    const float xf = __builtin_amdgcn_ldexpf(u, (int)x.lw) - 0.5f, yf = __builtin_amdgcn_ldexpf(v, (int)x.lh) - 0.5f;
    const float flx = floorf(xf), fly = floorf(yf);
    t.fx = xf - flx; t.fy = yf - fly;
    const uint32_t xi = (uint32_t)(int)flx, yi = (uint32_t)(int)fly;
    const uint32_t i0 = __builtin_amdgcn_ubfe(xi, 0u, x.lw), j0 = __builtin_amdgcn_ubfe(yi, 0u, x.lh), j1 = __builtin_amdgcn_ubfe(yi + 1u, 0u, x.lh);
    const uint32_t sh = x.lw + 2u, i0b = i0 << 2;
    const u32x2a4 p0 = gload64<u32x2a4>(x.base, (j0 << sh) | i0b), p1 = gload64<u32x2a4>(x.base, (j1 << sh) | i0b);
    t.t00 = p0.x; t.t10 = p0.y; t.t01 = p1.x; t.t11 = p1.y;
    if (__builtin_amdgcn_ubfe(xi + 1u, 0u, x.lw) == 0u) {
        t.t10 = gload64<uint32_t>(x.base, j0 << sh); t.t11 = gload64<uint32_t>(x.base, j1 << sh);
    }
}
struct Weights { float w00, w10, w01, w11; };
AWSM_DI Weights weights(const Tap& t) {
    const float gx = 1.0f - t.fx, gy = 1.0f - t.fy;
    return {gx * gy, t.fx * gy, gx * t.fy, t.fx * t.fy};
}
template <int BYTE> AWSM_DI float ub(uint32_t t) {
    return (float)((t >> (8 * BYTE)) & 255u);
}
template <int BYTE> AWSM_DI float channel(const Tap& t, const Weights& w) {
    return ub<BYTE>(t.t00) * w.w00 + ub<BYTE>(t.t10) * w.w10 + ub<BYTE>(t.t01) * w.w01 + ub<BYTE>(t.t11) * w.w11;
}
AWSM_DI f2 brdf_lut(const uint16_t* lut, uint32_t lut_w, uint32_t lut_h, float n_dot_v, float roughness) {
    const float u = saturate(n_dot_v), v = saturate(roughness);
    const int W = (int)lut_w, H = (int)lut_h;
    const float x = u * (float)W - 0.5f, y = v * (float)H - 0.5f;
    const float flx = floorf(x), fly = floorf(y);
    const float fx = x - flx, fy = y - fly;
    const int xi = (int)flx, yi = (int)fly;
    const int i0 = max(xi, 0), i1 = min(xi + 1, W - 1), j0 = max(yi, 0), j1 = min(yi + 1, H - 1);
    const uint32_t r0 = (uint32_t)(j0 * W) << 2, r1 = (uint32_t)(j1 * W) << 2;
    const uint32_t t00 = gload<uint32_t>(lut, r0 + ((uint32_t)i0 << 2)), t10 = gload<uint32_t>(lut, r0 + ((uint32_t)i1 << 2));
    const uint32_t t01 = gload<uint32_t>(lut, r1 + ((uint32_t)i0 << 2)), t11 = gload<uint32_t>(lut, r1 + ((uint32_t)i1 << 2));
    const float gx = 1.0f - fx, gy = 1.0f - fy;
    const float r_top = f16_bits_to_f32((unsigned short)(t00 & 0xFFFFu)) * gx + f16_bits_to_f32((unsigned short)(t10 & 0xFFFFu)) * fx;
    const float r_bot = f16_bits_to_f32((unsigned short)(t01 & 0xFFFFu)) * gx + f16_bits_to_f32((unsigned short)(t11 & 0xFFFFu)) * fx;
    const float g_top = f16_bits_to_f32((unsigned short)(t00 >> 16)) * gx + f16_bits_to_f32((unsigned short)(t10 >> 16)) * fx;
    const float g_bot = f16_bits_to_f32((unsigned short)(t01 >> 16)) * gx + f16_bits_to_f32((unsigned short)(t11 >> 16)) * fx;
    return {r_top * gy + r_bot * fy, g_top * gy + g_bot * fy};
}
struct Lit {
    f3 n, v, F0, df90, bd;
    float ndv_raw, ndv_dir, ndv4, a2m1, a2_g1v, gk, one_m_gk, occlusion, F0max, df90max;
};
AWSM_DI void direct(const Lit& s, f3 l, f3 radiance, f3& color) {
    const float ndl = saturate(fm::fdot(s.n, l));
#ifndef AWSM_NO_LIGHT_SKIP
    if (__builtin_amdgcn_ballot_w64(ndl > 0.0f) == 0ull) return;
#endif
    const f3 sum = s.v + l;
    const float len_sq = fm::fdot(sum, sum);
    const bool has_half = len_sq > 1e-8f;
    const float inv_len = has_half ? fm::rsq(len_sq) : 0.0f;
    const float ndh = saturate(fm::fdot(s.n, sum) * inv_len);
    const float vdh = fm::fdot(s.v, sum) * inv_len;
    const float p = saturate(1.0f - (has_half ? vdh : s.ndv_dir));
    const float p2 = p * p, p5 = (p2 * p2) * p;
    const f3 F = {s.F0.x + s.df90.x * p5, s.F0.y + s.df90.y * p5, s.F0.z + s.df90.z * p5};
    const float dd = (ndh * ndh) * s.a2m1 + 1.0f;
    const float den = (((kPi * dd) * dd + kEps) * (ndl * s.one_m_gk + s.gk)) * fmaxf(s.ndv4 * ndl, kEps);
    const float spec = has_half ? (s.a2_g1v * ndl) * fm::rcp(den) : 0.0f;
    const float k_d = 1.0f - (s.F0max + s.df90max * p5);
    const float w = ndl * s.occlusion;
    color.x += (s.bd.x * k_d + F.x * spec) * (radiance.x * w);
    color.y += (s.bd.y * k_d + F.y * spec) * (radiance.y * w);
    color.z += (s.bd.z * k_d + F.z * spec) * (radiance.z * w);
}
}

#ifndef AWSM_LEAN_SLOTS
#define AWSM_LEAN_SLOTS 16u
#endif
constexpr uint32_t kLeanSlots = AWSM_LEAN_SLOTS, kLeanChunks = 13u, kLeanNone = 0xFFFFFFFFu;
struct LeanStage { uint4 q[kLeanSlots][kLeanChunks]; };
#define AWSM_AS3 __attribute__((address_space(3)))
AWSM_DI float4 bits_float4(uint4 v) { return make_float4(__uint_as_float(v.x), __uint_as_float(v.y), __uint_as_float(v.z), __uint_as_float(v.w)); }
AWSM_DI double2 bits_double2(uint4 v) { return make_double2(__hiloint2double((int)v.y, (int)v.x), __hiloint2double((int)v.w, (int)v.z)); }
AWSM_DI uint4 as_uint4(u32x4 v) { return make_uint4(v.x, v.y, v.z, v.w); }

namespace lean {
struct TexS { const void* base; uint32_t lw, lh; };
AWSM_DI TexS decode_s(uint32_t lo, uint32_t hi) { return {reinterpret_cast<const void*>(((unsigned long long)(hi & 0xFFFFu) << 32) | lo), (hi >> 16) & 15u, (hi >> 20) & 15u}; }
AWSM_DI void fetch_s(const TexS& x, float u, float v, Tap& t) {
    const float xf = __builtin_amdgcn_ldexpf(u, (int)x.lw) - 0.5f, yf = __builtin_amdgcn_ldexpf(v, (int)x.lh) - 0.5f;
    const float flx = floorf(xf), fly = floorf(yf);
    t.fx = xf - flx; t.fy = yf - fly;
    const uint32_t xi = (uint32_t)(int)flx, yi = (uint32_t)(int)fly;
    const uint32_t i0 = __builtin_amdgcn_ubfe(xi, 0u, x.lw), j0 = __builtin_amdgcn_ubfe(yi, 0u, x.lh), j1 = __builtin_amdgcn_ubfe(yi + 1u, 0u, x.lh);
    const uint32_t sh = x.lw + 2u, i0b = i0 << 2;
    const u32x2a4 p0 = gload<u32x2a4>(x.base, (j0 << sh) | i0b), p1 = gload<u32x2a4>(x.base, (j1 << sh) | i0b);
    t.t00 = p0.x; t.t10 = p0.y; t.t01 = p1.x; t.t11 = p1.y;
    if (__builtin_amdgcn_ubfe(xi + 1u, 0u, x.lw) == 0u) {
        t.t10 = gload<uint32_t>(x.base, j0 << sh); t.t11 = gload<uint32_t>(x.base, j1 << sh);
    }
}
template <typename BASE> struct TexGT { BASE base; uint32_t lw, levels, layer, layers; };
typedef TexGT<const void*> TexG;
typedef TexGT<unsigned long long> TexGL;
AWSM_DI TexG decode_g(uint32_t w0, uint32_t w1, uint32_t w2, uint32_t w3) {
    return {reinterpret_cast<const void*>(((unsigned long long)(w1 & 0xFFFFu) << 32) | w0), w1 >> 24, (w1 >> 16) & 15u, w2, w3};
}
AWSM_DI TexGL decode_gl(uint32_t w0, uint32_t w1, uint32_t w2, uint32_t w3) {
    return {((unsigned long long)(w1 & 0xFFFFu) << 32) | w0, w1 >> 24, (w1 >> 16) & 15u, w2, w3};
}
template <typename T> AWSM_DI T gload_any(const void* base, uint32_t off) { return gload<T>(base, off); }
template <typename T> AWSM_DI T gload_any(unsigned long long base, uint32_t off) { return gload64<T>(base, off); }
struct Lod { uint32_t lo, hi; float f; };
template <typename BASE> AWSM_DI Lod select_lod(const TexGT<BASE>& x, float m2) {
    const float rho2 = __builtin_amdgcn_ldexpf(m2, (int)(2u * x.lw));
    float lod = 0.5f * __builtin_amdgcn_logf(fmaxf(rho2, 1e-12f));
    Lod r = {0u, 0u, 0.0f};
    if (lod > 0.0f && x.levels > 1u) {
        lod = fminf(lod, (float)(x.levels - 1u));
        const float fl = floorf(lod);
        r.lo = (uint32_t)fl; r.hi = min(r.lo + 1u, x.levels - 1u); r.f = (r.hi != r.lo) ? lod - fl : 0.0f;
    }
    return r;
}
template <typename BASE> AWSM_DI void fetch_g(const TexGT<BASE>& x, uint32_t level, float u, float v, Tap& t) {
    const uint32_t lwl = x.lw - level;
    const uint32_t g_all = __builtin_amdgcn_ubfe(0x55555555u, 0u, 2u * (x.lw + 1u)), g_rest = __builtin_amdgcn_ubfe(0x55555555u, 0u, 2u * (lwl + 1u));
    const uint32_t first = x.layers * (g_all - g_rest) + (x.layer << (2u * lwl));
    const float xf = __builtin_amdgcn_ldexpf(u, (int)lwl) - 0.5f, yf = __builtin_amdgcn_ldexpf(v, (int)lwl) - 0.5f;
    const float flx = floorf(xf), fly = floorf(yf);
    t.fx = xf - flx; t.fy = yf - fly;
    const uint32_t xi = (uint32_t)(int)flx, yi = (uint32_t)(int)fly;
    const uint32_t i0 = __builtin_amdgcn_ubfe(xi, 0u, lwl), j0 = __builtin_amdgcn_ubfe(yi, 0u, lwl), j1 = __builtin_amdgcn_ubfe(yi + 1u, 0u, lwl);
    const uint32_t r0 = (first + (j0 << lwl)) << 2, r1 = (first + (j1 << lwl)) << 2, i0b = i0 << 2;
    const u32x2a4 p0 = gload_any<u32x2a4>(x.base, r0 + i0b), p1 = gload_any<u32x2a4>(x.base, r1 + i0b);
    t.t00 = p0.x; t.t10 = p0.y; t.t01 = p1.x; t.t11 = p1.y;
    if (__builtin_amdgcn_ubfe(xi + 1u, 0u, lwl) == 0u) {
        t.t10 = gload_any<uint32_t>(x.base, r0); t.t11 = gload_any<uint32_t>(x.base, r1);
    }
}
AWSM_DI f4 cube_level_b(const void* base, const void* scene, uint32_t which, uint32_t size, uint32_t level, uint32_t face, float sn, float tn) {
    const uint32_t N = max(size >> level, 1u), P = N + 2u;
    const uint32_t lvl0 = gload<uint32_t>(scene, (uint32_t)(offsetof(DevScene, cube) + which * sizeof(CubeDev) + offsetof(CubeDev, b_level_off)) + level * 4u);
    float x = sn * (float)N - 0.5f, y = tn * (float)N - 0.5f;
    if (!(x >= -0.5f)) x = -0.5f;
    if (!(y >= -0.5f)) y = -0.5f;
    x = fminf(x, (float)N - 0.5f); y = fminf(y, (float)N - 0.5f);
    const float flx = floorf(x), fly = floorf(y), fx = x - flx, fy = y - fly;
    const uint32_t ib = (uint32_t)((int)flx + 1), jb = (uint32_t)((int)fly + 1);
    const uint32_t t0 = (lvl0 + (face * P + jb) * P + ib) << 3;
    typedef uint32_t u32x4a8 __attribute__((ext_vector_type(4), aligned(8)));
    const u32x4a8 r0 = gload<u32x4a8>(base, t0), r1 = gload<u32x4a8>(base, t0 + (P << 3));
    const f4 c00 = half4(make_uint2(r0.x, r0.y)), c10 = half4(make_uint2(r0.z, r0.w)), c01 = half4(make_uint2(r1.x, r1.y)), c11 = half4(make_uint2(r1.z, r1.w));
    return lerp4(lerp4(c00, c10, fx), lerp4(c01, c11, fx), fy);
}
template <uint32_t WHICH>
AWSM_DI f4 cube_sample(const DevScene* sc, f3 d, float level) {
    const uint32_t o = (uint32_t)(offsetof(DevScene, cube) + WHICH * sizeof(CubeDev));
    const u32x2 bp = cload<u32x2>(sc, o + (uint32_t)offsetof(CubeDev, bordered));
    const u32x2 sm = cload<u32x2>(sc, o + (uint32_t)offsetof(CubeDev, size));
    const void* base = reinterpret_cast<const void*>(((unsigned long long)bp.y << 32) | bp.x);
    const uint32_t size = sm.x, mips = sm.y;
    const float ax = fabsf(d.x), ay = fabsf(d.y), az = fabsf(d.z);
    uint32_t face; float scd, tcd, ma;
    if (az >= ax && az >= ay) { face = d.z < 0.0f ? 5u : 4u; scd = d.z < 0.0f ? -d.x : d.x; tcd = -d.y; ma = az; }
    else if (ay >= ax) { face = d.y < 0.0f ? 3u : 2u; scd = d.x; tcd = d.y < 0.0f ? -d.z : d.z; ma = ay; }
    else { face = d.x < 0.0f ? 1u : 0u; scd = d.x < 0.0f ? d.z : -d.z; tcd = -d.y; ma = ax; }
    const float inv = fm::rcp(ma);
    const float sn = 0.5f * (scd * inv) + 0.5f, tn = 0.5f * (tcd * inv) + 0.5f;
    const float top = (float)(mips - 1u);
    float lod = level > 0.0f ? level : 0.0f;
    lod = fminf(lod, top);
    const float fl = floorf(lod), fr = lod - fl;
    const uint32_t l0 = (uint32_t)fl, l1 = min(l0 + 1u, mips - 1u);
    f4 r = cube_level_b(base, sc, WHICH, size, l0, face, sn, tn);
    if (__builtin_amdgcn_ballot_w64(fr > 0.0f && l1 != l0) != 0ull) { const f4 h = cube_level_b(base, sc, WHICH, size, l1, face, sn, tn); if (fr > 0.0f && l1 != l0) r = lerp4(r, h, fr); }
    return r;
}
AWSM_DI f3 irradiance(const DevScene* sc, f3 n) {
    if (!sc->cube[kCubeIrradiance].bordered) return sample_irradiance(sc, n);
    const f4 c = cube_sample<kCubeIrradiance>(sc, n, 0.0f);
    return {c.x, c.y, c.z};
}
AWSM_DI f3 prefiltered(const DevScene* sc, f3 dir, float roughness) {
    if (!sc->cube[kCubePrefiltered].bordered) return sample_prefiltered(sc, dir, roughness);
    const uint32_t mip_count = cload<uint32_t>(sc->buf[AWSM_BUF_LIGHTS_INFO], 4u);
    const f4 c = cube_sample<kCubePrefiltered>(sc, dir, roughness * (float)(mip_count - 1u));
    return {c.x, c.y, c.z};
}
struct TapG { Tap lo, hi; float f; };
template <typename BASE> AWSM_DI void fetch_trilinear(const TexGT<BASE>& x, float m2, float u, float v, TapG& t) {
    const Lod l = select_lod(x, m2);
    t.f = l.f;
    fetch_g(x, l.lo, u, v, t.lo);
    if (__builtin_amdgcn_ballot_w64(l.f > 0.0f) != 0ull) fetch_g(x, l.hi, u, v, t.hi);
    else t.hi = t.lo;
}
template <int BYTE> AWSM_DI float channel(const TapG& t, const Weights& wl, const Weights& wh) {
    const float a = channel<BYTE>(t.lo, wl), b = channel<BYTE>(t.hi, wh);
    return a * (1.0f - t.f) + b * t.f;
}
struct Foot { uint32_t i0b, row0, row1, g_rest, sh2; bool wrap; };
AWSM_DI void footprint(uint32_t lwl, float u, float v, Foot& ft, float& fx, float& fy) {
    const float xf = __builtin_amdgcn_ldexpf(u, (int)lwl) - 0.5f, yf = __builtin_amdgcn_ldexpf(v, (int)lwl) - 0.5f;
    const float flx = floorf(xf), fly = floorf(yf);
    fx = xf - flx; fy = yf - fly;
    const uint32_t xi = (uint32_t)(int)flx, yi = (uint32_t)(int)fly;
    const uint32_t i0 = __builtin_amdgcn_ubfe(xi, 0u, lwl), j0 = __builtin_amdgcn_ubfe(yi, 0u, lwl), j1 = __builtin_amdgcn_ubfe(yi + 1u, 0u, lwl);
    ft.i0b = i0 << 2; ft.row0 = j0 << lwl; ft.row1 = j1 << lwl;
    ft.wrap = __builtin_amdgcn_ubfe(xi + 1u, 0u, lwl) == 0u;
    ft.g_rest = __builtin_amdgcn_ubfe(0x55555555u, 0u, 2u * (lwl + 1u)); ft.sh2 = 2u * lwl;
}
struct Quad { uint32_t t00, t10, t01, t11; };
template <typename BASE> AWSM_DI void fetch_q(const TexGT<BASE>& x, const Foot& ft, Quad& q) {
    const uint32_t g_all = __builtin_amdgcn_ubfe(0x55555555u, 0u, 2u * (x.lw + 1u));
    const uint32_t first = x.layers * (g_all - ft.g_rest) + (x.layer << ft.sh2);
    const uint32_t r0 = (first + ft.row0) << 2, r1 = (first + ft.row1) << 2;
    const u32x2a4 p0 = gload_any<u32x2a4>(x.base, r0 + ft.i0b), p1 = gload_any<u32x2a4>(x.base, r1 + ft.i0b);
    q.t00 = p0.x; q.t10 = p0.y; q.t01 = p1.x; q.t11 = p1.y;
    if (ft.wrap) { q.t10 = gload_any<uint32_t>(x.base, r0); q.t11 = gload_any<uint32_t>(x.base, r1); }
}
AWSM_DI TexG decode_any(const void*, uint32_t w0, uint32_t w1, uint32_t w2, uint32_t w3) { return decode_g(w0, w1, w2, w3); }
AWSM_DI TexGL decode_any(unsigned long long, uint32_t w0, uint32_t w1, uint32_t w2, uint32_t w3) { return decode_gl(w0, w1, w2, w3); }
struct W8 { float l00, l10, l01, l11, h00, h10, h01, h11; };
template <int BYTE> AWSM_DI float channel8(const Quad& lo, const Quad& hi, const W8& w) {
    return ((ub<BYTE>(lo.t00) * w.l00 + ub<BYTE>(lo.t10) * w.l10) + (ub<BYTE>(lo.t01) * w.l01 + ub<BYTE>(lo.t11) * w.l11)) +
           ((ub<BYTE>(hi.t00) * w.h00 + ub<BYTE>(hi.t10) * w.h10) + (ub<BYTE>(hi.t01) * w.h01 + ub<BYTE>(hi.t11) * w.h11));
}
}

struct LeanItem { int cx, cy; uint32_t rank; float depth; bool live; f3 color; };
template <int GRAD, bool MSAA, bool ITEMS>
AWSM_DI bool lean_core(const DevScene* __restrict__ sc, const FrameDev& f, const ShadeBlock& b, const uint32_t wg, const uint32_t tid, LeanStage* __restrict__ st, LeanItem* __restrict__ item) {
    const uint32_t lane = tid & 63u;
    const int cx = ITEMS ? item->cx : b.x0 + (int)(tid & 15u), cy = ITEMS ? item->cy : b.y0 + (int)(tid >> 4);
    const bool inside = ITEMS ? item->live : (cx < (int)f.width && cy < (int)f.sy1);
    const uint32_t pv = (uint32_t)cy * f.width + (uint32_t)cx;
    const uint32_t p = f.out_compact ? (((b.brow >> 1) << kTileShift) + ((uint32_t)cy & (uint32_t)(kTile - 1))) * f.width + (uint32_t)cx : pv;

    u32x2 key = {0xFFFFFFFFu, 0xFFFFFFFFu};
    bool want_c0 = false;
    if (ITEMS) { if (inside) key = {~item->rank, __float_as_uint(item->depth)}; }
    else if (!MSAA) { if (inside) key = gload<u32x2>(f.vis, pv << 3); }
    else {
        u32x4 ka = {0xFFFFFFFFu, 0xFFFFFFFFu, 0xFFFFFFFFu, 0xFFFFFFFFu}, kb = ka;
        if (inside) { ka = gload<u32x4>(f.vis, pv << 5); kb = gload<u32x4>(f.vis, (pv << 5) + 16u); }
        key = {ka.x, ka.y};
        const bool bg0 = (ka.x & ka.y) == 0xFFFFFFFFu, bg1 = (ka.z & ka.w) == 0xFFFFFFFFu, bg2 = (kb.x & kb.y) == 0xFFFFFFFFu, bg3 = (kb.z & kb.w) == 0xFFFFFFFFu;
        bool sure = false, test = false;
        if (!(bg0 && bg1 && bg2 && bg3)) {
            if (bg0) sure = true;
            else if (bg1 || bg2 || bg3 || ka.z != ka.x || kb.x != ka.x || kb.z != ka.x) {
                const m4 inv_proj = cload_m4(f.camera, 256u);
                const unsigned long long k4[4] = {((unsigned long long)ka.y << 32) | ka.x, ((unsigned long long)ka.w << 32) | ka.z, ((unsigned long long)kb.y << 32) | kb.x, ((unsigned long long)kb.w << 32) | kb.z};
                sure = edge_mask_depth_msaa_filtered(inv_proj, k4, (float)cx + 0.5f, (float)cy + 0.5f, (float)f.width, (float)f.height);
                test = !sure;
            }
        }
        const unsigned long long m_sure = __builtin_amdgcn_ballot_w64(sure), m_test = __builtin_amdgcn_ballot_w64(test);
        if (lane == 0u) *reinterpret_cast<ulonglong2*>(f.msaa_edge_bits + (size_t)(b.blk * 4u + (tid >> 6)) * 2u) = make_ulonglong2(m_sure, m_test);
        want_c0 = sure || test;
    }
    bool hud = false;
    if (!ITEMS && !MSAA && f.hud_vis && inside) { const u32x2 hk = gload<u32x2>(f.hud_vis, pv << 3); hud = (hk.x & hk.y) != 0xFFFFFFFFu; }
    if (hud) { store_pixel(f, p, f4{0.0f, 0.0f, 0.0f, 0.0f}); key = {0xFFFFFFFFu, 0xFFFFFFFFu}; }
    const bool hit = inside && (key.x & key.y) != 0xFFFFFFFFu;
    if (!ITEMS && inside && !hit && !hud) {
        const f4 sky = skybox_color(sc, f, cx, cy);
        store_pixel(f, p, sky);
        if (MSAA) {
            f.msaa_cells[pv] = make_uint2(0u, 0xFFFFFFFFu);
            if (want_c0) f.msaa_color0[pv] = make_float4(sky.x, sky.y, sky.z, sky.w);
        }
    }
    unsigned long long rem = __builtin_amdgcn_ballot_w64(hit);
    if (rem == 0ull) return true;
    const uint32_t rank = hit ? ~key.x : 0xFFFFFFFFu;
    const float depth = __uint_as_float(key.y);

    asm volatile("; MARK level1");
    unsigned long long src_base; uint32_t src_stride;
    {
        const uint32_t j = lane;
        const unsigned long long rec = (unsigned long long)f.tri_rec, nr = (unsigned long long)f.nrm, tn = (unsigned long long)f.tan, tsh = (unsigned long long)f.tri_shade;
        src_base = j < 5u ? rec + j * 16u : (j < 8u ? nr + (j - 5u) * 16u : (j < 11u ? tn + (j - 8u) * 16u : tsh + (j - 11u) * 16u));
        src_stride = j < 5u ? (uint32_t)kTriRecBytes : (j < 11u ? 48u : 32u);
    }
    uint32_t my_slot = kLeanNone, n_slots = 0u;
    while (rem != 0ull && n_slots < kLeanSlots) {
        const uint32_t r = (uint32_t)__builtin_amdgcn_readlane((int)rank, (int)__builtin_ctzll(rem));
        if (rank == r) my_slot = n_slots;
        if (lane < kLeanChunks)
            __builtin_amdgcn_global_load_lds((const AWSM_AS1 void*)(src_base + (unsigned long long)r * src_stride), (AWSM_AS3 void*)&st->q[n_slots][0], 16, 0, 0);
        rem &= ~__builtin_amdgcn_uicmp(rank, r, 32 );
        n_slots++;
    }
    asm volatile("s_waitcnt vmcnt(0)" ::: "memory");
    const bool staged = my_slot != kLeanNone;
    const uint4* rec = &st->q[staged ? my_slot : 0u][0];
    uint4 ts0 = rec[11], ts1 = rec[12];
    TriRecRaw raw;
    raw.q0 = bits_float4(rec[0]); raw.q1 = bits_float4(rec[1]); raw.q2 = bits_float4(rec[2]); raw.d3 = bits_double2(rec[3]); raw.d4 = bits_double2(rec[4]);
    float4 n0 = bits_float4(rec[5]), n1 = bits_float4(rec[6]), n2 = bits_float4(rec[7]);
    float4 t0 = bits_float4(rec[8]), t1 = bits_float4(rec[9]), t2 = bits_float4(rec[10]);
    if (hit && !staged) {
        ts0 = as_uint4(gload<u32x4>(f.tri_shade, rank << 5)); ts1 = as_uint4(gload<u32x4>(f.tri_shade, (rank << 5) + 16u));
        const uint32_t ro = rank * (uint32_t)kTriRecBytes, vo = rank * 48u;
        raw.q0 = as_float4(gload<f32x4>(f.tri_rec, ro)); raw.q1 = as_float4(gload<f32x4>(f.tri_rec, ro + 16u)); raw.q2 = as_float4(gload<f32x4>(f.tri_rec, ro + 32u));
        { const f64x2 a = gload<f64x2>(f.tri_rec, ro + 48u), c = gload<f64x2>(f.tri_rec, ro + 64u); raw.d3 = make_double2(a.x, a.y); raw.d4 = make_double2(c.x, c.y); }
        n0 = as_float4(gload<f32x4>(f.nrm, vo)); n1 = as_float4(gload<f32x4>(f.nrm, vo + 16u)); n2 = as_float4(gload<f32x4>(f.nrm, vo + 32u));
        t0 = as_float4(gload<f32x4>(f.tan, vo)); t1 = as_float4(gload<f32x4>(f.tan, vo + 16u)); t2 = as_float4(gload<f32x4>(f.tan, vo + 32u));
    }

    asm volatile("; MARK strict");
    TriSetup t;
    tri_rec_unpack(raw, t);
    const GBufferTexel g = reconstruct_core<(GRAD != 0)>(t, n0, n1, n2, t0, t1, t2, cx, cy);
    if (MSAA && hit) f.msaa_cells[pv] = make_uint2(oct_word(mk2(g.packed_nt.x, g.packed_nt.y)), key.y);
    const float bz = (1.0f - g.bx) - g.by;
    float u = interp3_strict(g.bx, g.by, bz, __uint_as_float(ts0.z), __uint_as_float(ts1.x), __uint_as_float(ts1.z));
    float v = interp3_strict(g.bx, g.by, bz, __uint_as_float(ts0.w), __uint_as_float(ts1.y), __uint_as_float(ts1.w));
    const uint32_t draw = ts0.x & 0x00FFFFFFu;
    const uint32_t d0 = (uint32_t)__builtin_amdgcn_readlane((int)draw, (int)__builtin_ctzll(__builtin_amdgcn_ballot_w64(hit)));
    const bool one_draw = __builtin_amdgcn_ballot_w64(hit && draw != d0) == 0ull;
    f2 ddx = {0.0f, 0.0f}, ddy = {0.0f, 0.0f};
    float m2 = 0.0f;
    float r2min = 0.0f; f2 major = {0.0f, 0.0f};
    if (GRAD) {
        const float x0 = __uint_as_float(ts0.z), y0 = __uint_as_float(ts0.w), x1 = __uint_as_float(ts1.x), y1 = __uint_as_float(ts1.y), x2 = __uint_as_float(ts1.z), y2 = __uint_as_float(ts1.w);
        const float dAlphaDx = g.bary_derivs.x, dAlphaDy = g.bary_derivs.y, dBetaDx = g.bary_derivs.z, dBetaDy = g.bary_derivs.w;
        const float dGammaDx = -dAlphaDx - dBetaDx, dGammaDy = -dAlphaDy - dBetaDy;
        ddx = {x0 * dAlphaDx + x1 * dBetaDx + x2 * dGammaDx, y0 * dAlphaDx + y1 * dBetaDx + y2 * dGammaDx};
        ddy = {x0 * dAlphaDy + x1 * dBetaDy + x2 * dGammaDy, y0 * dAlphaDy + y1 * dBetaDy + y2 * dGammaDy};
        const bool tiny = (fabsf(dAlphaDx) + fabsf(dAlphaDy) + fabsf(dBetaDx) + fabsf(dBetaDy)) < 1e-20f;
        const bool ok = (ddx.x == ddx.x) && (ddx.y == ddx.y) && (ddy.x == ddy.x) && (ddy.y == ddy.y);
        if (tiny || !ok) { ddx = {0.0f, 0.0f}; ddy = {0.0f, 0.0f}; }
    }
    if (GRAD == 0) {
    } else if (one_draw) {
        const uint32_t lo = d0 * (uint32_t)sizeof(LeanDrawDev);
        if (cload<uint32_t>(f.draw_lean, lo) & 8u) {
            const f32x4 ta = cload<f32x4>(f.draw_lean, lo + 176u); const f32x2a4 tb = cload<f32x2a4>(f.draw_lean, lo + 192u);
            const float u2 = affine2_strict(ta.x, ta.y, tb.x, u, v), v2 = affine2_strict(ta.z, ta.w, tb.y, u, v);
            u = u2; v = v2;
            if (GRAD) { ddx = {ta.x * ddx.x + ta.y * ddx.y, ta.z * ddx.x + ta.w * ddx.y}; ddy = {ta.x * ddy.x + ta.y * ddy.y, ta.z * ddy.x + ta.w * ddy.y}; }
        }
    } else {
        const uint32_t lo = draw * (uint32_t)sizeof(LeanDrawDev);
        const bool xf = (gload<uint32_t>(f.draw_lean, lo) & 8u) != 0u;
        if (__builtin_amdgcn_ballot_w64(xf) != 0ull) {
            const f32x4 ta = gload<f32x4>(f.draw_lean, lo + 176u); const f32x2a4 tb = gload<f32x2a4>(f.draw_lean, lo + 192u);
            const float u2 = affine2_strict(ta.x, ta.y, tb.x, u, v), v2 = affine2_strict(ta.z, ta.w, tb.y, u, v);
            if (xf) { u = u2; v = v2; }
            if (GRAD && xf) { ddx = {ta.x * ddx.x + ta.y * ddx.y, ta.z * ddx.x + ta.w * ddx.y}; ddy = {ta.x * ddy.x + ta.y * ddy.y, ta.z * ddy.x + ta.w * ddy.y}; }
        }
    }
    if (GRAD) {
        const float rx2 = ddx.x * ddx.x + ddx.y * ddx.y, ry2 = ddy.x * ddy.x + ddy.y * ddy.y;
        m2 = fmaxf(rx2, ry2);
        if (GRAD == 2) { r2min = fminf(rx2, ry2); major = rx2 >= ry2 ? ddx : ddy; }
    }
    bool todo = GRAD != 0 && __builtin_amdgcn_ballot_w64(hit && !(fabsf(u) <= 32768.0f && fabsf(v) <= 32768.0f)) != 0ull;

    asm volatile("; MARK fetch");
    f3 base, emissive;
    float metallic_in, roughness_in, normal_scale, occlusion_strength, normal_bias, occlusion_bias;
    uint32_t exists;
    lean::Tap tp0, tp1, tp2, tp3, tp4;
    lean::TapG tg0, tg1, tg2, tg3, tg4;
    constexpr uint32_t kNeed = GRAD == 2 ? 7u : (GRAD ? 3u : 1u);
    auto fetch_all = [&](float uu, float vv, float m2e, bool act, const uint32_t tex_mask = 31u, const bool factors = true) {
        if (one_draw) {
            const uint32_t lo = d0 * (uint32_t)sizeof(LeanDrawDev);
            const u32x4 L0 = cload<u32x4>(f.draw_lean, lo), L1 = cload<u32x4>(f.draw_lean, lo + 16u), L2 = cload<u32x4>(f.draw_lean, lo + 32u);
            const u32x4 L3 = cload<u32x4>(f.draw_lean, lo + 48u), L4 = cload<u32x4>(f.draw_lean, lo + 64u);
            const u32x2 L5 = cload<u32x2>(f.draw_lean, lo + 80u), L5s = cload<u32x2>(f.draw_lean, lo + 88u);
            if (GRAD == 0) {
                if (L0.x & 8u) {
                    const f32x4 ta = cload<f32x4>(f.draw_lean, lo + 176u); const f32x2a4 tb = cload<f32x2a4>(f.draw_lean, lo + 192u);
                    const float u2 = affine2_strict(ta.x, ta.y, tb.x, uu, vv), v2 = affine2_strict(ta.z, ta.w, tb.y, uu, vv);
                    uu = u2; vv = v2;
                }
                todo = todo || __builtin_amdgcn_ballot_w64(hit && !(fabsf(uu) <= 32768.0f && fabsf(vv) <= 32768.0f)) != 0ull;
            }
            todo = todo || (L0.x & kNeed) != kNeed;
            const uint32_t exs = todo ? 0u : L0.x >> 8;
            const uint32_t ex = act ? exs & tex_mask : 0u;
            if (GRAD) {
                const u32x4 G0 = cload<u32x4>(f.draw_lean, lo + 96u), G1 = cload<u32x4>(f.draw_lean, lo + 112u), G2 = cload<u32x4>(f.draw_lean, lo + 128u);
                const u32x4 G3 = cload<u32x4>(f.draw_lean, lo + 144u), G4 = cload<u32x4>(f.draw_lean, lo + 160u);
                if (ex & 1u) lean::fetch_trilinear(lean::decode_g(G0.x, G0.y, G0.z, G0.w), m2e, uu, vv, tg0);
                if (ex & 2u) lean::fetch_trilinear(lean::decode_g(G1.x, G1.y, G1.z, G1.w), m2e, uu, vv, tg1);
                if (ex & 4u) lean::fetch_trilinear(lean::decode_g(G2.x, G2.y, G2.z, G2.w), m2e, uu, vv, tg2);
                if (ex & 8u) lean::fetch_trilinear(lean::decode_g(G3.x, G3.y, G3.z, G3.w), m2e, uu, vv, tg3);
                if (ex & 16u) lean::fetch_trilinear(lean::decode_g(G4.x, G4.y, G4.z, G4.w), m2e, uu, vv, tg4);
            } else {
                if (ex & 1u) lean::fetch_s(lean::decode_s(L3.x, L3.y), uu, vv, tp0);
                if (ex & 2u) lean::fetch_s(lean::decode_s(L3.z, L3.w), uu, vv, tp1);
                if (ex & 4u) lean::fetch_s(lean::decode_s(L4.x, L4.y), uu, vv, tp2);
                if (ex & 8u) lean::fetch_s(lean::decode_s(L4.z, L4.w), uu, vv, tp3);
                if (ex & 16u) lean::fetch_s(lean::decode_s(L5.x, L5.y), uu, vv, tp4);
            }
            exists = exs;
            if (factors) {
            metallic_in = __uint_as_float(L0.y); roughness_in = __uint_as_float(L0.z); normal_scale = __uint_as_float(L0.w);
            base = {__uint_as_float(L1.x), __uint_as_float(L1.y), __uint_as_float(L1.z)}; occlusion_strength = __uint_as_float(L1.w);
            emissive = {__uint_as_float(L2.x), __uint_as_float(L2.y), __uint_as_float(L2.z)}; normal_bias = __uint_as_float(L2.w); occlusion_bias = __uint_as_float(L5s.x);
            }
        } else {
            const uint32_t lo = draw * (uint32_t)sizeof(LeanDrawDev);
            const u32x4 L0 = gload<u32x4>(f.draw_lean, lo), L1 = gload<u32x4>(f.draw_lean, lo + 16u), L2 = gload<u32x4>(f.draw_lean, lo + 32u);
            const u32x4 L3 = gload<u32x4>(f.draw_lean, lo + 48u), L4 = gload<u32x4>(f.draw_lean, lo + 64u);
            const u32x2 L5 = gload<u32x2>(f.draw_lean, lo + 80u), L5s = gload<u32x2>(f.draw_lean, lo + 88u);
            if (GRAD == 0) {
                if (__builtin_amdgcn_ballot_w64((L0.x & 8u) != 0u) != 0ull) {
                    const f32x4 ta = gload<f32x4>(f.draw_lean, lo + 176u); const f32x2a4 tb = gload<f32x2a4>(f.draw_lean, lo + 192u);
                    const float u2 = affine2_strict(ta.x, ta.y, tb.x, uu, vv), v2 = affine2_strict(ta.z, ta.w, tb.y, uu, vv);
                    if (L0.x & 8u) { uu = u2; vv = v2; }
                }
                todo = todo || __builtin_amdgcn_ballot_w64(hit && !(fabsf(uu) <= 32768.0f && fabsf(vv) <= 32768.0f)) != 0ull;
            }
            todo = todo || __builtin_amdgcn_ballot_w64(hit && (L0.x & kNeed) != kNeed) != 0ull;
            const uint32_t exs = (todo || !hit) ? 0u : L0.x >> 8;
            const uint32_t ex = act ? exs & tex_mask : 0u;
            if (GRAD) {
                const u32x4 G0 = gload<u32x4>(f.draw_lean, lo + 96u), G1 = gload<u32x4>(f.draw_lean, lo + 112u), G2 = gload<u32x4>(f.draw_lean, lo + 128u);
                const u32x4 G3 = gload<u32x4>(f.draw_lean, lo + 144u), G4 = gload<u32x4>(f.draw_lean, lo + 160u);
                if (ex & 1u) lean::fetch_trilinear(lean::decode_gl(G0.x, G0.y, G0.z, G0.w), m2e, uu, vv, tg0);
                if (ex & 2u) lean::fetch_trilinear(lean::decode_gl(G1.x, G1.y, G1.z, G1.w), m2e, uu, vv, tg1);
                if (ex & 4u) lean::fetch_trilinear(lean::decode_gl(G2.x, G2.y, G2.z, G2.w), m2e, uu, vv, tg2);
                if (ex & 8u) lean::fetch_trilinear(lean::decode_gl(G3.x, G3.y, G3.z, G3.w), m2e, uu, vv, tg3);
                if (ex & 16u) lean::fetch_trilinear(lean::decode_gl(G4.x, G4.y, G4.z, G4.w), m2e, uu, vv, tg4);
            } else {
                const lean::Tex x0 = lean::decode(L3.x, L3.y), x1 = lean::decode(L3.z, L3.w), x2 = lean::decode(L4.x, L4.y), x3 = lean::decode(L4.z, L4.w), x4 = lean::decode(L5.x, L5.y);
                if (ex & 1u) lean::fetch(x0, uu, vv, tp0);
                if (ex & 2u) lean::fetch(x1, uu, vv, tp1);
                if (ex & 4u) lean::fetch(x2, uu, vv, tp2);
                if (ex & 8u) lean::fetch(x3, uu, vv, tp3);
                if (ex & 16u) lean::fetch(x4, uu, vv, tp4);
            }
            exists = exs;
            if (factors) {
            metallic_in = __uint_as_float(L0.y); roughness_in = __uint_as_float(L0.z); normal_scale = __uint_as_float(L0.w);
            base = {__uint_as_float(L1.x), __uint_as_float(L1.y), __uint_as_float(L1.z)}; occlusion_strength = __uint_as_float(L1.w);
            emissive = {__uint_as_float(L2.x), __uint_as_float(L2.y), __uint_as_float(L2.z)}; normal_bias = __uint_as_float(L2.w); occlusion_bias = __uint_as_float(L5s.x);
            }
        }
    };
    float nf = 1.0f;
    if (GRAD == 2) {
        const uint32_t A = one_draw ? cload<uint32_t>(f.draw_lean, d0 * (uint32_t)sizeof(LeanDrawDev) + 92u) : gload<uint32_t>(f.draw_lean, draw * (uint32_t)sizeof(LeanDrawDev) + 92u);
        if (A > 1u && m2 > 0.0f) {
            const float Af = (float)min(A, 16u);
            nf = r2min * (Af * Af) <= m2 ? Af : __builtin_sqrtf(m2 / r2min);
            nf = fminf(fmaxf(nf, 1.0f), Af);
        }
    }
    const float m2c = GRAD == 2 ? m2 * fm::rcp(nf * nf) : m2;
    f3 world_position, surface_to_camera;
    TBN tbn;
    f3 normal;
    float occlusion = 1.0f;
    auto mid = [&]() {
    asm volatile("; MARK standard");
    const float pxf = (float)cx, pyf = (float)cy;
    const float* M = f.pix2view;
    const float hx = M[0] * pxf + (M[4] * pyf + (M[8] * depth + M[12])), hy = M[1] * pxf + (M[5] * pyf + (M[9] * depth + M[13]));
    const float hz = M[2] * pxf + (M[6] * pyf + (M[10] * depth + M[14])), hw = M[3] * pxf + (M[7] * pyf + (M[11] * depth + M[15]));
    const float ivw = fm::rcp(fmaxf(hw, 1e-8f));
    const f3 vp = {hx * ivw, hy * ivw, hz * ivw};
    const float* R = f.view_rot;
    const f3 rel = {R[0] * vp.x + (R[3] * vp.y + R[6] * vp.z), R[1] * vp.x + (R[4] * vp.y + R[7] * vp.z), R[2] * vp.x + (R[5] * vp.y + R[8] * vp.z)};
    world_position = {rel.x + f.cam_pos[0], rel.y + f.cam_pos[1], rel.z + f.cam_pos[2]};
#ifdef AWSM_STRICT_POSITION
    world_position = strict_world_position(cload_m4(f.camera, 256u), cload_m4(f.camera, 320u), cx, cy, (float)f.width, (float)f.height, depth);
#endif
    if (f.cam_ortho) {
        surface_to_camera = mk3(f.ortho_view_dir[0], f.ortho_view_dir[1], f.ortho_view_dir[2]);
    } else {
        const f3 to_camera = mk3(f.cam_pos[0], f.cam_pos[1], f.cam_pos[2]) - world_position;
        surface_to_camera = fm::fdot(to_camera, to_camera) > 0.0f ? fm::fsafe_normalize(to_camera) : mk3(0.0f, 0.0f, 1.0f);
    }
    asm volatile("; MARK tbn");
    tbn = fm::funpack_normal_tangent(g.packed_nt);
    normal = tbn.N;
    };
    bool shared_fp = false;
    float Lm = 0.0f;
    auto lean_word = [&](auto one, uint32_t off) {
        if constexpr (decltype(one)::value) return cload<uint32_t>(f.draw_lean, d0 * (uint32_t)sizeof(LeanDrawDev) + off);
        else return gload<uint32_t>(f.draw_lean, draw * (uint32_t)sizeof(LeanDrawDev) + off);
    };
    auto lean_quad = [&](auto one, uint32_t off) {
        if constexpr (decltype(one)::value) return cload<u32x4>(f.draw_lean, d0 * (uint32_t)sizeof(LeanDrawDev) + off);
        else return gload<u32x4>(f.draw_lean, draw * (uint32_t)sizeof(LeanDrawDev) + off);
    };
    auto decide = [&](auto one) {
        const uint32_t fl = lean_word(one, 0u);
        const uint32_t exs = (fl & kNeed) == kNeed ? (fl >> 8) & 31u : 0u;
        int lw_min = 15, top_min = 15;
#pragma unroll
        for (uint32_t k = 0; k < (uint32_t)kCoreTextures; k++) {
            const uint32_t w1 = lean_word(one, 96u + 16u * k + 4u);
            const int lw = (int)(w1 >> 24), lv = (int)((w1 >> 16) & 15u);
            if (exs & (1u << k)) { lw_min = min(lw_min, lw); top_min = min(top_min, lv - 1 - lw); }
        }
        Lm = 0.5f * __builtin_amdgcn_logf(fmaxf(m2c, 1e-30f));
        const bool in = exs != 0u && Lm > -(float)lw_min && Lm < (float)top_min;
        return __builtin_amdgcn_ballot_w64(hit && !in) == 0ull;
    };
    if (GRAD == 1 && !todo) shared_fp = one_draw ? decide(std::true_type{}) : decide(std::false_type{});
    auto shared_path = [&](auto one) {
        if constexpr (decltype(one)::value) asm volatile("; MARK fetch1"); else asm volatile("; MARK fetch1v");
        lean::W8 w8;
        lean::Quad ql0, qh0, ql1, qh1, ql2, qh2, ql3, qh3, ql4, qh4;
        const u32x4 L0 = lean_quad(one, 0u), L1 = lean_quad(one, 16u), L2 = lean_quad(one, 32u);
        const uint32_t L5s = lean_word(one, 88u);
        const u32x4 G0 = lean_quad(one, 96u), G1 = lean_quad(one, 112u), G2 = lean_quad(one, 128u), G3 = lean_quad(one, 144u), G4 = lean_quad(one, 160u);
        exists = hit ? (L0.x >> 8) & 31u : 0u;
        const float flL = floorf(Lm), ff = Lm - flL;
        const uint32_t cl = hit ? (uint32_t)(-(int)flL) : 1u;
        lean::Foot f_lo, f_hi;
        float fxl, fyl, fxh, fyh;
        lean::footprint(cl, u, v, f_lo, fxl, fyl);
        lean::footprint(cl - 1u, u, v, f_hi, fxh, fyh);
        typedef decltype(lean::decode_any(std::conditional_t<decltype(one)::value, const void*, unsigned long long>{}, 0u, 0u, 0u, 0u)) TexT;
        const std::conditional_t<decltype(one)::value, const void*, unsigned long long> tag{};
        if (exists & 1u) { const TexT x = lean::decode_any(tag, G0.x, G0.y, G0.z, G0.w); lean::fetch_q(x, f_lo, ql0); lean::fetch_q(x, f_hi, qh0); }
        if (exists & 2u) { const TexT x = lean::decode_any(tag, G1.x, G1.y, G1.z, G1.w); lean::fetch_q(x, f_lo, ql1); lean::fetch_q(x, f_hi, qh1); }
        if (exists & 4u) { const TexT x = lean::decode_any(tag, G2.x, G2.y, G2.z, G2.w); lean::fetch_q(x, f_lo, ql2); lean::fetch_q(x, f_hi, qh2); }
        if (exists & 8u) { const TexT x = lean::decode_any(tag, G3.x, G3.y, G3.z, G3.w); lean::fetch_q(x, f_lo, ql3); lean::fetch_q(x, f_hi, qh3); }
        if (exists & 16u) { const TexT x = lean::decode_any(tag, G4.x, G4.y, G4.z, G4.w); lean::fetch_q(x, f_lo, ql4); lean::fetch_q(x, f_hi, qh4); }
        metallic_in = __uint_as_float(L0.y); roughness_in = __uint_as_float(L0.z); normal_scale = __uint_as_float(L0.w);
        base = {__uint_as_float(L1.x), __uint_as_float(L1.y), __uint_as_float(L1.z)}; occlusion_strength = __uint_as_float(L1.w);
        emissive = {__uint_as_float(L2.x), __uint_as_float(L2.y), __uint_as_float(L2.z)}; normal_bias = __uint_as_float(L2.w); occlusion_bias = __uint_as_float(L5s);
        const float gl = 1.0f - ff, gxl = 1.0f - fxl, gyl = 1.0f - fyl, gxh = 1.0f - fxh, gyh = 1.0f - fyh;
        const float a = gyl * gl, b = fyl * gl, c = gyh * ff, d = fyh * ff;
        w8 = {gxl * a, fxl * a, gxl * b, fxl * b, gxh * c, fxh * c, gxh * d, fxh * d};
        if (!hit) return false;
        mid();
        if constexpr (decltype(one)::value) asm volatile("; MARK material1"); else asm volatile("; MARK material1v");
        if (exists & 1u) base = {base.x * lean::channel8<0>(ql0, qh0, w8), base.y * lean::channel8<1>(ql0, qh0, w8), base.z * lean::channel8<2>(ql0, qh0, w8)};
        if (exists & 2u) { metallic_in = metallic_in * lean::channel8<2>(ql1, qh1, w8); roughness_in = roughness_in * lean::channel8<1>(ql1, qh1, w8); }
        if (exists & 4u) {
            const float ntx = lean::channel8<0>(ql2, qh2, w8) * normal_scale - normal_bias, nty = lean::channel8<1>(ql2, qh2, w8) * normal_scale - normal_bias, ntz = lean::channel8<2>(ql2, qh2, w8) * (2.0f / 255.0f) - 1.0f;
            normal = fm::fnormalize(tbn.T * ntx + tbn.B * nty + tbn.N * ntz);
        }
        if (exists & 8u) occlusion = lean::channel8<0>(ql3, qh3, w8) * occlusion_strength + occlusion_bias;
        if (exists & 16u) emissive = {emissive.x * lean::channel8<0>(ql4, qh4, w8), emissive.y * lean::channel8<1>(ql4, qh4, w8), emissive.z * lean::channel8<2>(ql4, qh4, w8)};
        return true;
    };
    if (GRAD == 1 && shared_fp) {
        if (!(one_draw ? shared_path(std::true_type{}) : shared_path(std::false_type{}))) return true;
    } else {
    fetch_all(u, v, m2c, true, GRAD == 1 ? 7u : 31u);
    if (todo) {
        if (!ITEMS && lane == 0u) {
            const uint32_t slot = atomicAdd(&f.shade_todo[0], 1u);
            if (slot < f.shade_todo_cap) f.shade_todo[4u + slot] = (wg << 2) | (tid >> 6);
        }
        return false;
    }
    if (!hit) return true;

    float ch[12] = {0.0f, 0.0f, 0.0f, 0.0f, 0.0f, 0.0f, 0.0f, 0.0f, 0.0f, 0.0f, 0.0f, 0.0f};
    if (GRAD == 2) {
#define AWSM_LEAN_ACC(I, K, BYTE) ch[I] += lean::channel<BYTE>(tg##K, wl, wh) * wj
        auto accumulate = [&](float wj) {
// ... 13 lines not shown
            const float inv_n = fm::rcp(nf);
            float wsum = 1.0f;
            for (int j = 1; j <= wave_m; j++) { const float tj = (float)j * inv_n, wj = saturate((0.5f - tj) * nf + 0.5f); wsum += 2.0f * wj; }
            auto probes = [&](const auto& tex, const bool has, auto&& acc) {
                if (__builtin_amdgcn_ballot_w64(has) == 0ull) return;
#pragma unroll 1
                for (int j = 1; j <= wave_m; j++) {
                    const float tj = (float)j * inv_n, wj = saturate((0.5f - tj) * nf + 0.5f);
                    const bool act = has && wj > 0.0f;
                    if (__builtin_amdgcn_ballot_w64(act) == 0ull) break;
                    if (act) {
                        lean::TapG ta, tb;
                        const float tn = -tj;
                        lean::fetch_trilinear(tex, m2c, u + major.x * tj, v + major.y * tj, ta);
                        lean::fetch_trilinear(tex, m2c, u + major.x * tn, v + major.y * tn, tb);
                        acc(ta, wj); acc(tb, wj);
                    }
                }
            };
#define AWSM_LEAN_ACC(I, BYTE) ch[I] += lean::channel<BYTE>(t, wl, wh) * wj
            auto acc0 = [&](const lean::TapG& t, float wj) { const lean::Weights wl = lean::weights(t.lo), wh = lean::weights(t.hi); AWSM_LEAN_ACC(0, 0); AWSM_LEAN_ACC(1, 1); AWSM_LEAN_ACC(2, 2); };
            auto acc1 = [&](const lean::TapG& t, float wj) { const lean::Weights wl = lean::weights(t.lo), wh = lean::weights(t.hi); AWSM_LEAN_ACC(3, 2); AWSM_LEAN_ACC(4, 1); };
            auto acc2 = [&](const lean::TapG& t, float wj) { const lean::Weights wl = lean::weights(t.lo), wh = lean::weights(t.hi); AWSM_LEAN_ACC(5, 0); AWSM_LEAN_ACC(6, 1); AWSM_LEAN_ACC(7, 2); };
            auto acc3 = [&](const lean::TapG& t, float wj) { const lean::Weights wl = lean::weights(t.lo), wh = lean::weights(t.hi); AWSM_LEAN_ACC(8, 0); };
            auto acc4 = [&](const lean::TapG& t, float wj) { const lean::Weights wl = lean::weights(t.lo), wh = lean::weights(t.hi); AWSM_LEAN_ACC(9, 0); AWSM_LEAN_ACC(10, 1); AWSM_LEAN_ACC(11, 2); };
#undef AWSM_LEAN_ACC
            if (one_draw) {
                const uint32_t lo = d0 * (uint32_t)sizeof(LeanDrawDev);
#define AWSM_LEAN_PROBE_TEX(K, ACC) { const u32x4 G = cload<u32x4>(f.draw_lean, lo + 96u + 16u * K); probes(lean::decode_g(G.x, G.y, G.z, G.w), (exists & (1u << K)) != 0u, ACC); }
                AWSM_LEAN_PROBE_TEX(0, acc0) AWSM_LEAN_PROBE_TEX(1, acc1) AWSM_LEAN_PROBE_TEX(2, acc2) AWSM_LEAN_PROBE_TEX(3, acc3) AWSM_LEAN_PROBE_TEX(4, acc4)
#undef AWSM_LEAN_PROBE_TEX
            } else {
                const uint32_t lo = draw * (uint32_t)sizeof(LeanDrawDev);
#define AWSM_LEAN_PROBE_TEX(K, ACC) { const u32x4 G = gload<u32x4>(f.draw_lean, lo + 96u + 16u * K); probes(lean::decode_gl(G.x, G.y, G.z, G.w), (exists & (1u << K)) != 0u, ACC); }
                AWSM_LEAN_PROBE_TEX(0, acc0) AWSM_LEAN_PROBE_TEX(1, acc1) AWSM_LEAN_PROBE_TEX(2, acc2) AWSM_LEAN_PROBE_TEX(3, acc3) AWSM_LEAN_PROBE_TEX(4, acc4)
#undef AWSM_LEAN_PROBE_TEX
            }
            const float iw = fm::rcp(wsum);
#pragma unroll
            for (int i = 0; i < 12; i++) ch[i] *= iw;
        }
    }

    mid();

    asm volatile("; MARK material");
#define AWSM_LEAN_TEX(K, W0, W1) const lean::Weights W0 = lean::weights(GRAD ? tg##K.lo : tp##K), W1 = lean::weights(GRAD ? tg##K.hi : tp##K)
#define AWSM_LEAN_CH(K, BYTE, W0, W1) (GRAD ? lean::channel<BYTE>(tg##K, W0, W1) : lean::channel<BYTE>(tp##K, W0))
    if (GRAD != 2) {
        if (exists & 1u) { AWSM_LEAN_TEX(0, w, wh); base = {base.x * AWSM_LEAN_CH(0, 0, w, wh), base.y * AWSM_LEAN_CH(0, 1, w, wh), base.z * AWSM_LEAN_CH(0, 2, w, wh)}; }
        if (exists & 2u) { AWSM_LEAN_TEX(1, w, wh); metallic_in = metallic_in * AWSM_LEAN_CH(1, 2, w, wh); roughness_in = roughness_in * AWSM_LEAN_CH(1, 1, w, wh); }
        if (exists & 4u) {
            AWSM_LEAN_TEX(2, w, wh);
            const float ntx = AWSM_LEAN_CH(2, 0, w, wh) * normal_scale - normal_bias, nty = AWSM_LEAN_CH(2, 1, w, wh) * normal_scale - normal_bias, ntz = AWSM_LEAN_CH(2, 2, w, wh) * (2.0f / 255.0f) - 1.0f;
            normal = fm::fnormalize(tbn.T * ntx + tbn.B * nty + tbn.N * ntz);
        }
        if (GRAD == 1 && __builtin_amdgcn_ballot_w64((exists & 24u) != 0u) != 0ull) fetch_all(u, v, m2c, true, 24u, false);
        if (exists & 8u) { AWSM_LEAN_TEX(3, w, wh); occlusion = AWSM_LEAN_CH(3, 0, w, wh) * occlusion_strength + occlusion_bias; }
        if (exists & 16u) { AWSM_LEAN_TEX(4, w, wh); emissive = {emissive.x * AWSM_LEAN_CH(4, 0, w, wh), emissive.y * AWSM_LEAN_CH(4, 1, w, wh), emissive.z * AWSM_LEAN_CH(4, 2, w, wh)}; }
    } else {
        if (exists & 1u) base = {base.x * ch[0], base.y * ch[1], base.z * ch[2]};
        if (exists & 2u) { metallic_in = metallic_in * ch[3]; roughness_in = roughness_in * ch[4]; }
        if (exists & 4u) {
            const float ntx = ch[5] * normal_scale - normal_bias, nty = ch[6] * normal_scale - normal_bias, ntz = ch[7] * (2.0f / 255.0f) - 1.0f;
            normal = fm::fnormalize(tbn.T * ntx + tbn.B * nty + tbn.N * ntz);
        }
        if (exists & 8u) occlusion = ch[8] * occlusion_strength + occlusion_bias;
        if (exists & 16u) emissive = {emissive.x * ch[9], emissive.y * ch[10], emissive.z * ch[11]};
    }
#undef AWSM_LEAN_TEX
#undef AWSM_LEAN_CH
    }

    asm volatile("; MARK surface");
    Surface sf;
    sf.n = fm::fsafe_normalize(normal);
    sf.v = fm::fsafe_normalize(surface_to_camera);
    sf.metallic = clampf(metallic_in, 0.0f, 1.0f);
    sf.roughness = fmaxf(clampf(roughness_in, 0.0f, 1.0f), 0.04f);
    sf.alpha = sf.roughness * sf.roughness;
    const float ndv = fm::fdot(sf.n, sf.v);
    sf.n_dot_v_ibl = saturate(ndv);
    sf.n_dot_v_dir = fmaxf(ndv, 1e-4f);
    const float f0b = ior_to_f0(1.5f);
    sf.F0 = mix3(splat3(fminf(f0b, 1.0f)), base, sf.metallic);
    sf.f90 = mixf(1.0f, 1.0f, sf.metallic);
    sf.sheen_scaling_dir = 1.0f;
    sf.g1_v = geometry_schlick_ggx(saturate(ndv), sf.alpha);
    sf.cc_n = sf.n;
    sf.df90 = splat3(sf.f90) - sf.F0;
    sf.base_diffuse = base * ((1.0f - sf.metallic) * (1.0f / kPi));
    const float ac = fmaxf(sf.alpha, 0.001f);
    sf.a2 = ac * ac; sf.a2m1 = sf.a2 - 1.0f;
    sf.gk = ((ac + 1.0f) * (ac + 1.0f)) * 0.125f; sf.one_m_gk = 1.0f - sf.gk;
    sf.has_sheen = false; sf.has_clearcoat = false;
    lean::Lit lit;
    lit.n = sf.n; lit.v = sf.v; lit.F0 = sf.F0; lit.df90 = sf.df90; lit.bd = sf.base_diffuse;
    lit.ndv_raw = ndv; lit.F0max = fmaxf(fmaxf(sf.F0.x, sf.F0.y), sf.F0.z); lit.df90max = sf.f90 - lit.F0max;
    lit.ndv_dir = sf.n_dot_v_dir; lit.ndv4 = 4.0f * sf.n_dot_v_dir; lit.a2m1 = sf.a2m1; lit.a2_g1v = sf.a2 * sf.g1_v; lit.gk = sf.gk; lit.one_m_gk = sf.one_m_gk;
    lit.occlusion = occlusion;
    f3 color;
    asm volatile("; MARK ibl");
    {
        const f3 prefiltered = lean::prefiltered(sc, reflect3(-sf.v, sf.n), sf.roughness);
        const f3 irradiance = lean::irradiance(sc, sf.n);
        const float n_dot_v = sf.n_dot_v_ibl;
        const f3 F_view = fresnel_schlick_f90(n_dot_v, sf.F0, sf.f90);
        const float F_view_max = fmaxf(fmaxf(F_view.x, F_view.y), F_view.z);
        const f3 base_layer = (base * (1.0f / kPi)) * irradiance;
        const float k_d = (1.0f - F_view_max) * (1.0f - sf.metallic);
        const f3 base_contribution = (base_layer * k_d) * occlusion;
        const f2 lut = lean::brdf_lut(sc->lut_rg16f, sc->lut_w, sc->lut_h, n_dot_v, sf.roughness);
        const f3 spec_term = sf.F0 * lut.x + splat3(sf.f90 * lut.y);
        const f3 specular = (prefiltered * spec_term) * mixf(1.0f, occlusion, 0.5f);
        color = (base_contribution + specular) + emissive;
    }
    asm volatile("; MARK lights");
    const uint32_t n_lights = min(cload<uint32_t>(sc->buf[AWSM_BUF_LIGHTS_INFO], 0u), f.lights_cap);
    const void* lights = sc->buf[AWSM_BUF_LIGHTS];
    for (uint32_t i = 0; i < n_lights; i++) {
        const f32x4 pre0 = cload<f32x4>(f.lights_pre, i * 32u), pre1 = cload<f32x4>(f.lights_pre, i * 32u + 16u);
        const uint32_t kind = (uint32_t)pre0.w;
        f3 light_dir = {pre0.x, pre0.y, pre0.z}, radiance = {pre1.x, pre1.y, pre1.z};
        if (kind == 2u || kind == 3u) {
            const f32x4 pos_range = cload<f32x4>(lights, i * 64u);
            const f3 stl = mk3(pos_range.x, pos_range.y, pos_range.z) - world_position;
            const float d2 = fm::fdot(stl, stl);
            const float inv_d = d2 > 0.0f ? fm::rsq(d2) : 0.0f;
            const float dist = d2 * inv_d;
            float att;
            if (pos_range.w == 0.0f) att = fm::rcp(fmaxf(dist * dist, 0.01f));
            else { const float fo = 1.0f - fm::fdiv(dist * dist, pos_range.w * pos_range.w); att = fm::fdiv(saturate(fo * fo), dist * dist + 1.0f); }
            const f3 to_light = stl * inv_d;
            if (kind == 3u) {
                const f32x4 dir_inner = cload<f32x4>(lights, i * 64u + 16u), kind_outer = cload<f32x4>(lights, i * 64u + 48u);
                const float cos_l = fm::fdot(to_light, -light_dir);
                const float sm = saturate(fm::fdiv(cos_l - kind_outer.y, dir_inner.w - kind_outer.y));
                att = att * (sm * sm);
            }
            light_dir = to_light;
            radiance = radiance * att;
#ifndef AWSM_NO_LIGHT_SKIP
            if (__builtin_amdgcn_ballot_w64(!(att == 0.0f)) == 0ull) continue;
#endif
        } else if (kind != 1u) { light_dir = {0.0f, 0.0f, 0.0f}; radiance = {0.0f, 0.0f, 0.0f}; }
        lean::direct(lit, light_dir, radiance, color);
    }
    asm volatile("; MARK store");
    if (ITEMS) { item->color = color; return true; }
    store_pixel(f, p, {color.x, color.y, color.z, 1.0f});
    if (MSAA && want_c0) f.msaa_color0[pv] = make_float4(color.x, color.y, color.z, 1.0f);
    return true;
}
template <int GRAD, bool MSAA>
AWSM_DI void lean_block(const DevScene* __restrict__ sc, const FrameDev& f, const ShadeBlock& b, const uint32_t wg, const uint32_t tid, LeanStage* __restrict__ st) {
    (void)lean_core<GRAD, MSAA, false>(sc, f, b, wg, tid, st, nullptr);
}
#ifndef AWSM_ANISO_WAVES
#define AWSM_ANISO_WAVES 4
#endif
#ifndef AWSM_LEAN_COUNTERS
#define AWSM_LEAN_COUNTERS 8
#endif
constexpr uint32_t kLeanCounters = AWSM_LEAN_COUNTERS;
#ifndef AWSM_LEAN_GRAD_WAVES
#define AWSM_LEAN_GRAD_WAVES 5
#endif
template <bool PERSIST, int GRAD, bool MSAA>
__global__ __launch_bounds__(256) __attribute__((amdgpu_waves_per_eu(GRAD == 2 ? AWSM_ANISO_WAVES : (GRAD ? AWSM_LEAN_GRAD_WAVES : (PERSIST ? 5 : AWSM_LEAN_WAVES))))) void k_shade_lean(const DevScene* __restrict__ sc, FrameDev f) {
    __shared__ LeanStage stage[4];
    if (frame_poisoned(f)) return;
#ifdef AWSM_LEAN_PRIO
    __builtin_amdgcn_s_setprio(AWSM_LEAN_PRIO);
#endif
    LeanStage* const st = &stage[__builtin_amdgcn_readfirstlane((int)(threadIdx.x >> 6))];
    const uint32_t xcd = blockIdx.x & 7u, lane = threadIdx.x & 63u;
    const uint32_t bx_n = (f.width + 15u) >> 4, by_n = f.band_n > 1u ? 2u * f.tiles_y : ((f.sy1 - f.sy0) + 15u) >> 4;
    const uint32_t lp = 32u - (uint32_t)__builtin_clz((bx_n - 1u) | 1u);
    const uint32_t share = (((by_n + 7u - xcd) >> 3) << lp) * 4u;
    const uint32_t w = __builtin_amdgcn_readfirstlane((blockIdx.x >> 3) * 4u + (threadIdx.x >> 6));
    uint32_t zero;
    asm volatile("v_mov_b32 %0, 0" : "=v"(zero));
    uint32_t c = w % kLeanCounters, tried = 0u;
    uint32_t* ctr0 = f.lean_next + (xcd * kLeanCounters) * 16u + zero;
    uint32_t nxt = 0u;
    if (PERSIST && lane == 0u) nxt = atomicAdd(ctr0 + c * 16u, 1u);
    for (uint32_t j = w;;) {
        if (PERSIST) {
            j = __builtin_amdgcn_readfirstlane(nxt) * kLeanCounters + c;
            while (j >= share && ++tried < kLeanCounters) {
                c = (c + 1u) % kLeanCounters;
                if (lane == 0u) nxt = atomicAdd(ctr0 + c * 16u, 1u);
                j = __builtin_amdgcn_readfirstlane(nxt) * kLeanCounters + c;
            }
            if (j >= share) break;
            if (lane == 0u) nxt = atomicAdd(ctr0 + c * 16u, 1u);
        }
        const uint32_t kb = j >> 2, bcol = kb & ((1u << lp) - 1u), brow = (kb >> lp) * 8u + xcd;
        if (bcol < bx_n && j < share) {
            ShadeBlock b;
            shade_block_at(f, b, brow, bcol);
            lean_block<GRAD, MSAA>(sc, f, b, ((kb >> lp) * bx_n + bcol) * 8u + xcd, ((j & 3u) << 6) | lane, st);
        }
        if (!PERSIST) break;
    }
}

constexpr uint32_t kEdgeRecBytes = 260;
struct NeighbourCell { float nx, ny, nz; uint32_t depth_bits; uint32_t state; };

AWSM_DI void publish_cell(NeighbourCell* cells, int lx, int ly, const FrameDev& f, int px, int py) {
    NeighbourCell c = {0.0f, 0.0f, 0.0f, 0u, 0u};
    if (px >= 0 && px < (int)f.width && py >= (int)f.y0 && py < (int)f.y1) {
        unsigned long long k;
        if (f.band_n > 1u && (((uint32_t)py >> kTileShift) % f.band_n) != f.band_r) {
            const uint32_t ty = (uint32_t)py >> kTileShift, which = ((uint32_t)py & (uint32_t)(kTile - 1)) == 0u ? 0u : 1u;
            k = f.msaa_halo ? f.msaa_halo[((((size_t)(ty % f.band_n) * f.halo_bands + ty / f.band_n) * 2u + which) * f.width) + (size_t)px] : ~0ull;
        } else k = f.vis[((size_t)py * f.width + (size_t)px) * 4];
        c.state = 1u;
        if (k != ~0ull) {
            const f3 n = strict_normal_of(f, key_rank(k), px, py);
            c.nx = n.x; c.ny = n.y; c.nz = n.z; c.depth_bits = (uint32_t)(k >> 32); c.state = 2u;
        }
    }
    cells[(ly + 1) * 18 + (lx + 1)] = c;
}

template <typename CellAt>
AWSM_DI bool edge_by_neighbours(const m4& inv_proj, f3 center_normal, float center_depth, float pcx, float pcy, float W, float H, CellAt cell) {
    bool is_edge = false, center_loaded = false;
    float view_depth_c = 0.0f, depth_threshold = 0.0f;
#pragma unroll
    for (int i = 0; i < 4; i++) {
        const int ox = i == 0 ? 1 : (i == 1 ? -1 : 0), oy = i == 2 ? 1 : (i == 3 ? -1 : 0);
        if (is_edge) continue;
        const NeighbourCell nb = cell(ox, oy);
        if (nb.state == 0u) continue;
        if (nb.state == 1u) { is_edge = true; continue; }
        if (dot(center_normal, mk3(nb.nx, nb.ny, nb.nz)) < kEdgeNormalThreshold) { is_edge = true; continue; }
        if (!center_loaded) {
            view_depth_c = view_space_depth(inv_proj, center_depth, pcx, pcy, W, H);
            depth_threshold = kEdgeDepthThreshold * fabsf(view_depth_c);
            center_loaded = true;
        }
        const float nvd = view_space_depth(inv_proj, __uint_as_float(nb.depth_bits), pcx + (float)ox, pcy + (float)oy, W, H);
        if (fabsf(view_depth_c - nvd) > depth_threshold) is_edge = true;
    }
    return is_edge;
}

AWSM_DI uint2 halo_cell(const FrameDev& f, int px, int py) {
    unsigned long long k;
    if (f.band_n > 1u && (((uint32_t)py >> kTileShift) % f.band_n) != f.band_r) {
        const uint32_t ty = (uint32_t)py >> kTileShift, which = ((uint32_t)py & (uint32_t)(kTile - 1)) == 0u ? 0u : 1u;
        k = f.msaa_halo ? f.msaa_halo[((((size_t)(ty % f.band_n) * f.halo_bands + ty / f.band_n) * 2u + which) * f.width) + (size_t)px] : ~0ull;
    } else k = f.vis[((size_t)py * f.width + (size_t)px) * 4];
    if (k == ~0ull) return make_uint2(0u, 0xFFFFFFFFu);
    return make_uint2(oct_word(strict_oct_of(f, key_rank(k), px, py)), (uint32_t)(k >> 32));
}
AWSM_DI bool detect_pixel(const FrameDev& f, const ShadeBlock& b, uint32_t slot, const m4& inv_proj, bool fastp) {
    const int cx = b.x0 + (int)(slot & 15u), cy = b.y0 + (int)(slot >> 4);
    uint2 nb[4];
    uint32_t state[4];
#pragma unroll
    for (int i = 0; i < 4; i++) {
        const int px = cx + (i == 0 ? 1 : (i == 1 ? -1 : 0)), py = cy + (i == 2 ? 1 : (i == 3 ? -1 : 0));
        nb[i] = make_uint2(0u, 0xFFFFFFFFu); state[i] = 0u;
        if (px >= 0 && px < (int)f.width && py >= (int)f.y0 && py < (int)f.y1) {
            if (i < 2 || row_owned(f, py)) { nb[i] = f.msaa_cells[(size_t)py * f.width + (size_t)px]; state[i] = 1u; }
            else state[i] = 2u;
        }
    }
    const uint2 me = f.msaa_cells[(size_t)cy * f.width + (size_t)cx];
    const float W = (float)f.width, H = (float)f.height, pcx = (float)cx + 0.5f, pcy = (float)cy + 0.5f;
    const f2 oct_c = oct_of_word(me.x);
    const f3 nc = fm::fdecode_octahedral(oct_c);
    const float dc = __uint_as_float(me.y);
    const float vdc = fastp ? view_depth_approx(inv_proj, dc) : view_space_depth(inv_proj, dc, pcx, pcy, W, H);
    bool is_edge = false;
#pragma unroll
    for (int i = 0; i < 4; i++) {
        const int ox = i == 0 ? 1 : (i == 1 ? -1 : 0), oy = i == 2 ? 1 : (i == 3 ? -1 : 0);
        if (is_edge || state[i] == 0u) continue;
        uint2 c = nb[i];
        if (state[i] == 2u) c = halo_cell(f, cx + ox, cy + oy);
// ... 449 lines not shown
```

Measured before the change: 3440 frames/s.

## Batch scalar loads for draw, IBL tail, lights and poison gate in lean shader

Adds a per-frame LeanTailDev record, filled by the resolve kernel, that packs light count, IBL cube modes, mip count, LUT dimensions and pointers. The lean shader now issues wide s_load batches early and waits only where the data is used: draw records, the tail record, software-pipelined per-light loads and a deferred poison check. The goal is to hide scalar-memory latency that previously serialized the shader's IBL and light loops. In exchange it relies on hand-written inline asm with manual lgkmcnt waits and adds a new buffer, which makes correctness fragile.

Result: slower. 3367 frames/s (-2.1%).

```diff
diff --git a/awsm-renderer_amd/csrc/awsm_hip.cpp b/awsm-renderer_amd/csrc/awsm_hip.cpp
--- a/awsm-renderer_amd/csrc/awsm_hip.cpp
+++ b/awsm-renderer_amd/csrc/awsm_hip.cpp
@@ -259,7 +259,7 @@
     f->draw_shade = (DrawShadeDev*)FB(c).draw_shade.ptr;
     f->tex_slots = (TexSlotDev*)FB(c).tex_slots.ptr;
     f->draw_mat = (DrawMatDev*)FB(c).draw_mat.ptr;
-    const bool lean_ok = !(c->flags & AWSM_CFG_GENERAL_SHADE_ONLY) && (uint64_t)c->width * c->height * (c->msaa == 4 ? 32u : 8u) < (1ull << 32) && (c->msaa == 0 || (c->msaa_edge_bits[c->slot].ptr && c->msaa_cells[c->slot].ptr)) && FB(c).tri_shade.ptr && FB(c).draw_lean.ptr && c->shade_todo[c->slot].ptr && ((uint64_t)world.total_tris + (view.merged ? hud.total_tris : 0u)) * kTriRecBytes < (1ull << 32) &&
+    const bool lean_ok = !(c->flags & AWSM_CFG_GENERAL_SHADE_ONLY) && (uint64_t)c->width * c->height * (c->msaa == 4 ? 32u : 8u) < (1ull << 32) && (c->msaa == 0 || (c->msaa_edge_bits[c->slot].ptr && c->msaa_cells[c->slot].ptr)) && FB(c).tri_shade.ptr && FB(c).draw_lean.ptr && c->shade_todo[c->slot].ptr && c->lean_tail[c->slot].ptr && ((uint64_t)world.total_tris + (view.merged ? hud.total_tris : 0u)) * kTriRecBytes < (1ull << 32) &&
                          c->bufs[AWSM_BUF_ATTR_DATA].size < (1ull << 32) - 64;
     f->tri_shade = lean_ok ? (uint4*)FB(c).tri_shade.ptr : nullptr;
     f->attr_data_bytes = (uint32_t)std::min<size_t>(c->bufs[AWSM_BUF_ATTR_DATA].size, 0xFFFFFFFFu);
@@ -304,6 +304,7 @@
     f->out_rgba32f = (float*)c->out32[c->slot].ptr;
     f->lights_pre = (float4*)c->lights_pre[c->slot].ptr;
     f->lights_cap = (uint32_t)(c->lights_pre[c->slot].size / 32);
+    f->lean_tail = lean_ok ? (LeanTailDev*)c->lean_tail[c->slot].ptr : nullptr;
 }
 
 void compose_pixel_to_view(AwsmHipCtx* c, FrameBufs& b) {
@@ -335,7 +336,7 @@
     AwsmHipCtx::ResolveKey k;
     memset(&k, 0, sizeof k);
     k.write_seq = c->write_seq + (c->scene_dirty ? 1u : 0u); k.draws_version = FB(c).draws_version;
-    k.ptrs[0] = f.draw_shade; k.ptrs[1] = f.draw_mat; k.ptrs[2] = f.tex_slots; k.ptrs[3] = f.draw_lean; k.ptrs[4] = f.lights_pre;
+    k.ptrs[0] = f.draw_shade; k.ptrs[1] = f.draw_mat; k.ptrs[2] = f.tex_slots; k.ptrs[3] = f.draw_lean; k.ptrs[4] = f.lights_pre; k.ptrs[5] = f.lean_tail;
     k.n_draws = f.n_draws; k.mipmap = c->last_opaque.mipmap; k.has_opaque = c->last_opaque.has_opaque; k.lights_cap = f.lights_cap;
     return k;
 }
@@ -904,7 +905,7 @@
     for (auto& b : c->merged_vis) fr(b);
     fr(c->pose_records);
     fr(c->env_stage); fr(c->env_tables); fr(c->env_rows); fr(c->env_filter_tab); if (c->ev_env_copy) (void)hipEventDestroy(c->ev_env_copy);
-    fr(c->lut); for (auto& b : c->cube_tex) fr(b); for (auto& b : c->cube_bordered) fr(b); fr(c->digest); for (auto& b : c->shade_todo) fr(b); for (int sl = 0; sl < kSlots; sl++) { fr(c->msaa_color0[sl]); fr(c->msaa_edges[sl]); fr(c->msaa_edge_bits[sl]); fr(c->msaa_cells[sl]); } fr(c->mip_kinds); for (auto& b : c->out16) fr(b); for (auto& b : c->out32) fr(b); fr(c->comp16); fr(c->comp32); fr(c->grid_layer); for (auto& b : c->lights_pre) fr(b);
+    fr(c->lut); for (auto& b : c->cube_tex) fr(b); for (auto& b : c->cube_bordered) fr(b); fr(c->digest); for (auto& b : c->shade_todo) fr(b); for (int sl = 0; sl < kSlots; sl++) { fr(c->msaa_color0[sl]); fr(c->msaa_edges[sl]); fr(c->msaa_edge_bits[sl]); fr(c->msaa_cells[sl]); } fr(c->mip_kinds); for (auto& b : c->out16) fr(b); for (auto& b : c->out32) fr(b); fr(c->comp16); fr(c->comp32); fr(c->grid_layer); for (auto& b : c->lights_pre) fr(b); for (auto& b : c->lean_tail) fr(b);
     for (auto& b : c->ssao_layers) fr(b);
     for (auto& b : c->taa_img) fr(b); fr(c->taa_layers);
     for (auto& b : c->sel_tables) fr(b);
@@ -1077,6 +1078,7 @@
     }
     c->msaa = msaa;
     for (int sl = 0; sl < n_slots(c); sl++) if ((rc = dev_realloc(c, c->shade_todo[sl], ((size_t)((width + 15) / 16) * ((height + 15) / 16) * 4 + 4 + 1024) * 4, true))) return rc;
+    for (int sl = 0; sl < n_slots(c); sl++) if (!c->lean_tail[sl].ptr && (rc = dev_realloc(c, c->lean_tail[sl], sizeof(LeanTailDev), true))) return rc;
     for (int sl = 0; sl < n_slots(c); sl++) {
         if ((rc = dev_realloc(c, c->out16[sl], px * 8, true))) return rc;
         if ((c->flags & AWSM_CFG_PARITY_TAP) && (rc = dev_realloc(c, c->out32[sl], px * 16, true))) return rc;
diff --git a/awsm-renderer_amd/csrc/ctx.hpp b/awsm-renderer_amd/csrc/ctx.hpp
--- a/awsm-renderer_amd/csrc/ctx.hpp
+++ b/awsm-renderer_amd/csrc/ctx.hpp
@@ -118,7 +118,7 @@
     hipStream_t shade_streams[kSlots] = {};
     bool shade_recorded[kSlots] = {};
     bool uploads_recorded[kSlots] = {};
-    struct ResolveKey { uint64_t write_seq, draws_version; const void* ptrs[5]; uint32_t n_draws, mipmap, has_opaque, lights_cap; } resolved[kSlots] = {};
+    struct ResolveKey { uint64_t write_seq, draws_version; const void* ptrs[6]; uint32_t n_draws, mipmap, has_opaque, lights_cap; } resolved[kSlots] = {};
     hipEvent_t ev_geom_done[kSlots] = {}, ev_shade_done[kSlots] = {}, ev_uploads[kSlots] = {} ;
     hipEvent_t ev_flush = nullptr;
     uint64_t write_seq = 0, geom_write_seq[kSlots] = {};
@@ -164,6 +164,7 @@
     bool post_done = false;
     AwsmPostParams post_params{};
     DevBuf lights_pre[kSlots];
+    DevBuf lean_tail[kSlots];
     void* bound_comp = nullptr;
     size_t bound_comp_bytes = 0;
     const void* msaa_halo = nullptr;
diff --git a/awsm-renderer_amd/csrc/frame_params.hpp b/awsm-renderer_amd/csrc/frame_params.hpp
--- a/awsm-renderer_amd/csrc/frame_params.hpp
+++ b/awsm-renderer_amd/csrc/frame_params.hpp
@@ -72,6 +72,17 @@
     uint32_t pad2[2];
 };
 static_assert(sizeof(LeanDrawDev) == 208, "LeanDrawDev must be 208 bytes");
+
+struct LeanTailDev {
+    uint32_t n_lights;
+    uint32_t pre_mode, irr_mode;
+    uint32_t pre_mips;
+    float pre_rgb[3]; uint32_t lut_w;
+    float irr_rgb[3]; uint32_t lut_h;
+    const uint8_t* lights;
+    const uint16_t* lut_rg16f;
+};
+static_assert(sizeof(LeanTailDev) == 64, "LeanTailDev must be 64 bytes");
 
 constexpr int kMaxMipLevels = 16;
 struct TexArrayDev {
@@ -138,6 +149,7 @@
     DrawMatDev* draw_mat;
     float4* lights_pre;
     uint32_t lights_cap;
+    LeanTailDev* lean_tail;
     float4* clip;
     float4* nrm;
     float4* tan;
diff --git a/awsm-renderer_amd/csrc/kernels_shade.hip b/awsm-renderer_amd/csrc/kernels_shade.hip
--- a/awsm-renderer_amd/csrc/kernels_shade.hip
+++ b/awsm-renderer_amd/csrc/kernels_shade.hip
@@ -298,6 +298,18 @@
             f.lights_pre[i * 2] = make_float4(v.x, v.y, v.z, kind_outer.x);
             f.lights_pre[i * 2 + 1] = make_float4(color_intensity.x * color_intensity.w, color_intensity.y * color_intensity.w, color_intensity.z * color_intensity.w, 0.0f);
         }
+    }
+    if (d == 0u && f.lean_tail) {
+        const uint32_t* info = reinterpret_cast<const uint32_t*>(sc->buf[AWSM_BUF_LIGHTS_INFO]);
+        const CubeDev& pc = sc->cube[kCubePrefiltered]; const CubeDev& ic = sc->cube[kCubeIrradiance];
+        LeanTailDev t;
+        t.n_lights = info ? min(info[0], f.lights_cap) : 0u;
+        t.pre_mode = pc.bordered ? 1u : (pc.texels ? 2u : 0u); t.irr_mode = ic.bordered ? 1u : (ic.texels ? 2u : 0u);
+        t.pre_mips = info ? info[1] : 0u;
+        for (int j = 0; j < 3; j++) { t.pre_rgb[j] = sc->prefiltered_rgb[j]; t.irr_rgb[j] = sc->irradiance_rgb[j]; }
+        t.lut_w = sc->lut_w; t.lut_h = sc->lut_h;
+        t.lights = sc->buf[AWSM_BUF_LIGHTS]; t.lut_rg16f = sc->lut_rg16f;
+        *f.lean_tail = t;
     }
     if (d == 0u && f.shade_todo) f.shade_todo[0] = 0u;
     if (d < 64u && f.lean_next) f.lean_next[d * 16u] = 0u;
@@ -1112,6 +1124,17 @@
 template <typename T> AWSM_DI T gload(const void* base, uint32_t byte_off) { return *(const AWSM_AS1 T*)((const AWSM_AS1 char*)base + byte_off); }
 template <typename T> AWSM_DI T gload64(unsigned long long base, uint32_t byte_off) { return *(const AWSM_AS1 T*)((const AWSM_AS1 char*)base + byte_off); }
 template <typename T> AWSM_DI T cload(const void* base, uint32_t byte_off) { return *(const AWSM_AS4 T*)((const AWSM_AS4 char*)base + byte_off); }
+typedef uint32_t u32x8 __attribute__((ext_vector_type(8)));
+typedef uint32_t u32x16 __attribute__((ext_vector_type(16)));
+template <typename T> struct SBatch;
+template <> struct SBatch<u32x4> { static AWSM_DI u32x4 issue(const void* base, uint32_t off) { u32x4 v; asm volatile("s_load_dwordx4 %0, %1, %2" : "=&s"(v) : "s"(base), "s"(off)); return v; } };
+template <> struct SBatch<u32x8> { static AWSM_DI u32x8 issue(const void* base, uint32_t off) { u32x8 v; asm volatile("s_load_dwordx8 %0, %1, %2" : "=&s"(v) : "s"(base), "s"(off)); return v; } };
+template <> struct SBatch<u32x16> { static AWSM_DI u32x16 issue(const void* base, uint32_t off) { u32x16 v; asm volatile("s_load_dwordx16 %0, %1, %2" : "=&s"(v) : "s"(base), "s"(off)); return v; } };
+template <> struct SBatch<uint32_t> { static AWSM_DI uint32_t issue(const void* base, uint32_t off) { uint32_t v; asm volatile("s_load_dword %0, %1, %2" : "=&s"(v) : "s"(base), "s"(off)); return v; } };
+template <typename A> AWSM_DI void swait(A& a) { asm volatile("s_waitcnt lgkmcnt(0)" : "+s"(a)); }
+template <typename A, typename B> AWSM_DI void swait(A& a, B& b) { asm volatile("s_waitcnt lgkmcnt(0)" : "+s"(a), "+s"(b)); }
+template <typename A, typename B, typename C> AWSM_DI void swait(A& a, B& b, C& c) { asm volatile("s_waitcnt lgkmcnt(0)" : "+s"(a), "+s"(b), "+s"(c)); }
+template <typename A, typename B, typename C, typename D> AWSM_DI void swait(A& a, B& b, C& c, D& d) { asm volatile("s_waitcnt lgkmcnt(0)" : "+s"(a), "+s"(b), "+s"(c), "+s"(d)); }
 AWSM_DI float4 as_float4(f32x4 v) { return make_float4(v.x, v.y, v.z, v.w); }
 AWSM_DI m4 cload_m4(const void* base, uint32_t byte_off) {
     m4 m;
@@ -1148,7 +1171,8 @@
 template <int BYTE> AWSM_DI float channel(const Tap& t, const Weights& w) {
     return ub<BYTE>(t.t00) * w.w00 + ub<BYTE>(t.t10) * w.w10 + ub<BYTE>(t.t01) * w.w01 + ub<BYTE>(t.t11) * w.w11;
 }
-AWSM_DI f2 brdf_lut(const uint16_t* lut, uint32_t lut_w, uint32_t lut_h, float n_dot_v, float roughness) {
+struct LutTaps { uint32_t t00, t10, t01, t11; float fx, fy; };
+AWSM_DI LutTaps lut_taps(const uint16_t* lut, uint32_t lut_w, uint32_t lut_h, float n_dot_v, float roughness) {
     const float u = saturate(n_dot_v), v = saturate(roughness);
     const int W = (int)lut_w, H = (int)lut_h;
     const float x = u * (float)W - 0.5f, y = v * (float)H - 0.5f;
@@ -1159,6 +1183,11 @@
     const uint32_t r0 = (uint32_t)(j0 * W) << 2, r1 = (uint32_t)(j1 * W) << 2;
     const uint32_t t00 = gload<uint32_t>(lut, r0 + ((uint32_t)i0 << 2)), t10 = gload<uint32_t>(lut, r0 + ((uint32_t)i1 << 2));
     const uint32_t t01 = gload<uint32_t>(lut, r1 + ((uint32_t)i0 << 2)), t11 = gload<uint32_t>(lut, r1 + ((uint32_t)i1 << 2));
+    return {t00, t10, t01, t11, fx, fy};
+}
+AWSM_DI f2 lut_blend(const LutTaps& t) {
+    const uint32_t t00 = t.t00, t10 = t.t10, t01 = t.t01, t11 = t.t11;
+    const float fx = t.fx, fy = t.fy;
     const float gx = 1.0f - fx, gy = 1.0f - fy;
     const float r_top = f16_bits_to_f32((unsigned short)(t00 & 0xFFFFu)) * gx + f16_bits_to_f32((unsigned short)(t10 & 0xFFFFu)) * fx;
     const float r_bot = f16_bits_to_f32((unsigned short)(t01 & 0xFFFFu)) * gx + f16_bits_to_f32((unsigned short)(t11 & 0xFFFFu)) * fx;
@@ -1298,14 +1327,13 @@
     if (__builtin_amdgcn_ballot_w64(fr > 0.0f && l1 != l0) != 0ull) { const f4 h = cube_level_b(base, sc, WHICH, size, l1, face, sn, tn); if (fr > 0.0f && l1 != l0) r = lerp4(r, h, fr); }
     return r;
 }
-AWSM_DI f3 irradiance(const DevScene* sc, f3 n) {
-    if (!sc->cube[kCubeIrradiance].bordered) return sample_irradiance(sc, n);
+AWSM_DI f3 irradiance(const DevScene* sc, f3 n, uint32_t mode) {
+    if (mode != 1u) return sample_irradiance(sc, n);
     const f4 c = cube_sample<kCubeIrradiance>(sc, n, 0.0f);
     return {c.x, c.y, c.z};
 }
-AWSM_DI f3 prefiltered(const DevScene* sc, f3 dir, float roughness) {
-    if (!sc->cube[kCubePrefiltered].bordered) return sample_prefiltered(sc, dir, roughness);
-    const uint32_t mip_count = cload<uint32_t>(sc->buf[AWSM_BUF_LIGHTS_INFO], 4u);
+AWSM_DI f3 prefiltered(const DevScene* sc, f3 dir, float roughness, uint32_t mode, uint32_t mip_count) {
+    if (mode != 1u) return sample_prefiltered(sc, dir, roughness);
     const f4 c = cube_sample<kCubePrefiltered>(sc, dir, roughness * (float)(mip_count - 1u));
     return {c.x, c.y, c.z};
 }
@@ -1351,21 +1379,29 @@
 }
 
 struct LeanItem { int cx, cy; uint32_t rank; float depth; bool live; f3 color; };
+struct LeanGate { bool pending, armed; uint32_t word; };
 template <int GRAD, bool MSAA, bool ITEMS>
-AWSM_DI bool lean_core(const DevScene* __restrict__ sc, const FrameDev& f, const ShadeBlock& b, const uint32_t wg, const uint32_t tid, LeanStage* __restrict__ st, LeanItem* __restrict__ item) {
+AWSM_DI bool lean_core(const DevScene* __restrict__ sc, const FrameDev& f, const ShadeBlock& b, const uint32_t wg, const uint32_t tid, LeanStage* __restrict__ st, LeanItem* __restrict__ item, const LeanGate gate = {false, false, 0u}) {
     const uint32_t lane = tid & 63u;
     const int cx = ITEMS ? item->cx : b.x0 + (int)(tid & 15u), cy = ITEMS ? item->cy : b.y0 + (int)(tid >> 4);
     const bool inside = ITEMS ? item->live : (cx < (int)f.width && cy < (int)f.sy1);
     const uint32_t pv = (uint32_t)cy * f.width + (uint32_t)cx;
     const uint32_t p = f.out_compact ? (((b.brow >> 1) << kTileShift) + ((uint32_t)cy & (uint32_t)(kTile - 1))) * f.width + (uint32_t)cx : pv;
 
+    auto gate_poisoned = [&]() {
+        if (ITEMS || !gate.pending) return false;
+        uint32_t w = gate.word;
+        swait(w);
+        return gate.armed && w == f.frame_serial;
+    };
     u32x2 key = {0xFFFFFFFFu, 0xFFFFFFFFu};
     bool want_c0 = false;
     if (ITEMS) { if (inside) key = {~item->rank, __float_as_uint(item->depth)}; }
-    else if (!MSAA) { if (inside) key = gload<u32x2>(f.vis, pv << 3); }
+    else if (!MSAA) { if (inside) key = gload<u32x2>(f.vis, pv << 3); if (gate_poisoned()) return true; }
     else {
         u32x4 ka = {0xFFFFFFFFu, 0xFFFFFFFFu, 0xFFFFFFFFu, 0xFFFFFFFFu}, kb = ka;
         if (inside) { ka = gload<u32x4>(f.vis, pv << 5); kb = gload<u32x4>(f.vis, (pv << 5) + 16u); }
+        if (gate_poisoned()) return true;
         key = {ka.x, ka.y};
         const bool bg0 = (ka.x & ka.y) == 0xFFFFFFFFu, bg1 = (ka.z & ka.w) == 0xFFFFFFFFu, bg2 = (kb.x & kb.y) == 0xFFFFFFFFu, bg3 = (kb.z & kb.w) == 0xFFFFFFFFu;
         bool sure = false, test = false;
@@ -1433,6 +1469,15 @@
         t0 = as_float4(gload<f32x4>(f.tan, vo)); t1 = as_float4(gload<f32x4>(f.tan, vo + 16u)); t2 = as_float4(gload<f32x4>(f.tan, vo + 32u));
     }
 
+    const uint32_t draw = ts0.x & 0x00FFFFFFu;
+    const uint32_t d0 = (uint32_t)__builtin_amdgcn_readlane((int)draw, (int)__builtin_ctzll(__builtin_amdgcn_ballot_w64(hit)));
+    const bool one_draw = __builtin_amdgcn_ballot_w64(hit && draw != d0) == 0ull;
+    u32x16 dr_a; u32x8 dr_b, dr_t;
+    if (GRAD == 0 && one_draw) {
+        const uint32_t lo = d0 * (uint32_t)sizeof(LeanDrawDev);
+        dr_a = SBatch<u32x16>::issue(f.draw_lean, lo); dr_b = SBatch<u32x8>::issue(f.draw_lean, lo + 64u); dr_t = SBatch<u32x8>::issue(f.draw_lean, lo + 176u);
+    }
+
     asm volatile("; MARK strict");
     TriSetup t;
     tri_rec_unpack(raw, t);
@@ -1441,9 +1486,6 @@
     const float bz = (1.0f - g.bx) - g.by;
     float u = interp3_strict(g.bx, g.by, bz, __uint_as_float(ts0.z), __uint_as_float(ts1.x), __uint_as_float(ts1.z));
     float v = interp3_strict(g.bx, g.by, bz, __uint_as_float(ts0.w), __uint_as_float(ts1.y), __uint_as_float(ts1.w));
-    const uint32_t draw = ts0.x & 0x00FFFFFFu;
-    const uint32_t d0 = (uint32_t)__builtin_amdgcn_readlane((int)draw, (int)__builtin_ctzll(__builtin_amdgcn_ballot_w64(hit)));
-    const bool one_draw = __builtin_amdgcn_ballot_w64(hit && draw != d0) == 0ull;
     f2 ddx = {0.0f, 0.0f}, ddy = {0.0f, 0.0f};
     float m2 = 0.0f;
     float r2min = 0.0f; f2 major = {0.0f, 0.0f};
@@ -1493,12 +1535,19 @@
     auto fetch_all = [&](float uu, float vv, float m2e, bool act, const uint32_t tex_mask = 31u, const bool factors = true) {
         if (one_draw) {
             const uint32_t lo = d0 * (uint32_t)sizeof(LeanDrawDev);
-            const u32x4 L0 = cload<u32x4>(f.draw_lean, lo), L1 = cload<u32x4>(f.draw_lean, lo + 16u), L2 = cload<u32x4>(f.draw_lean, lo + 32u);
-            const u32x4 L3 = cload<u32x4>(f.draw_lean, lo + 48u), L4 = cload<u32x4>(f.draw_lean, lo + 64u);
-            const u32x2 L5 = cload<u32x2>(f.draw_lean, lo + 80u), L5s = cload<u32x2>(f.draw_lean, lo + 88u);
+            u32x4 L0, L1, L2, L3, L4; u32x2 L5, L5s;
+            if (GRAD == 0) {
+                swait(dr_a, dr_b, dr_t);
+                L0 = {dr_a[0], dr_a[1], dr_a[2], dr_a[3]}; L1 = {dr_a[4], dr_a[5], dr_a[6], dr_a[7]}; L2 = {dr_a[8], dr_a[9], dr_a[10], dr_a[11]}; L3 = {dr_a[12], dr_a[13], dr_a[14], dr_a[15]};
+                L4 = {dr_b[0], dr_b[1], dr_b[2], dr_b[3]}; L5 = {dr_b[4], dr_b[5]}; L5s = {dr_b[6], dr_b[7]};
+            } else {
+                L0 = cload<u32x4>(f.draw_lean, lo); L1 = cload<u32x4>(f.draw_lean, lo + 16u); L2 = cload<u32x4>(f.draw_lean, lo + 32u);
+                L3 = cload<u32x4>(f.draw_lean, lo + 48u); L4 = cload<u32x4>(f.draw_lean, lo + 64u);
+                L5 = cload<u32x2>(f.draw_lean, lo + 80u); L5s = cload<u32x2>(f.draw_lean, lo + 88u);
+            }
             if (GRAD == 0) {
                 if (L0.x & 8u) {
-                    const f32x4 ta = cload<f32x4>(f.draw_lean, lo + 176u); const f32x2a4 tb = cload<f32x2a4>(f.draw_lean, lo + 192u);
+                    const f32x4 ta = {__uint_as_float(dr_t[0]), __uint_as_float(dr_t[1]), __uint_as_float(dr_t[2]), __uint_as_float(dr_t[3])}; const f32x2a4 tb = {__uint_as_float(dr_t[4]), __uint_as_float(dr_t[5])};
                     const float u2 = affine2_strict(ta.x, ta.y, tb.x, uu, vv), v2 = affine2_strict(ta.z, ta.w, tb.y, uu, vv);
                     uu = u2; vv = v2;
                 }
@@ -1582,6 +1631,7 @@
     TBN tbn;
     f3 normal;
     float occlusion = 1.0f;
+    u32x16 tail;
     auto mid = [&]() {
     asm volatile("; MARK standard");
     const float pxf = (float)cx, pyf = (float)cy;
@@ -1602,9 +1652,11 @@
         const f3 to_camera = mk3(f.cam_pos[0], f.cam_pos[1], f.cam_pos[2]) - world_position;
         surface_to_camera = fm::fdot(to_camera, to_camera) > 0.0f ? fm::fsafe_normalize(to_camera) : mk3(0.0f, 0.0f, 1.0f);
     }
+    tail = SBatch<u32x16>::issue(f.lean_tail, 0u);
     asm volatile("; MARK tbn");
     tbn = fm::funpack_normal_tangent(g.packed_nt);
     normal = tbn.N;
+    swait(tail);
     };
     bool shared_fp = false;
     float Lm = 0.0f;
@@ -1784,6 +1836,34 @@
     const float ndv = fm::fdot(sf.n, sf.v);
     sf.n_dot_v_ibl = saturate(ndv);
     sf.n_dot_v_dir = fmaxf(ndv, 1e-4f);
+    f3 color;
+    asm volatile("; MARK ibl");
+    f3 prefiltered = {__uint_as_float(tail[4]), __uint_as_float(tail[5]), __uint_as_float(tail[6])};
+    if (tail[1] != 0u) prefiltered = lean::prefiltered(sc, reflect3(-sf.v, sf.n), sf.roughness, tail[1], tail[3]);
+    f3 irradiance = {__uint_as_float(tail[8]), __uint_as_float(tail[9]), __uint_as_float(tail[10])};
+    if (tail[2] != 0u) irradiance = lean::irradiance(sc, sf.n, tail[2]);
+    const lean::LutTaps taps = lean::lut_taps(reinterpret_cast<const uint16_t*>(((unsigned long long)tail[15] << 32) | tail[14]), tail[7], tail[11], sf.n_dot_v_ibl, sf.roughness);
+    uint32_t n_lights, lights_lo, lights_hi;
+    asm("s_mov_b32 %0, %3\n\ts_mov_b32 %1, %4\n\ts_mov_b32 %2, %5" : "=&s"(n_lights), "=&s"(lights_lo), "=&s"(lights_hi) : "s"(tail[0]), "s"(tail[12]), "s"(tail[13]));
+    const void* lights = reinterpret_cast<const void*>(((unsigned long long)lights_hi << 32) | lights_lo);
+    struct LightRaw { u32x8 p; u32x4 q; uint32_t inner, outer; };
+    struct LightRec { f32x4 pre0, pre1, pos_range; float cos_inner, cos_outer; };
+    auto light_issue = [](const void* pre, const void* rec, uint32_t i) {
+        LightRaw r;
+        r.p = SBatch<u32x8>::issue(pre, i * 32u); r.q = SBatch<u32x4>::issue(rec, i * 64u);
+        r.inner = SBatch<uint32_t>::issue(rec, i * 64u + 28u); r.outer = SBatch<uint32_t>::issue(rec, i * 64u + 52u);
+        return r;
+    };
+    auto light_wait = [](LightRaw& r) { swait(r.p, r.q, r.inner, r.outer); };
+    auto light_unpack = [](const LightRaw& r) {
+        LightRec l;
+        l.pre0 = {__uint_as_float(r.p[0]), __uint_as_float(r.p[1]), __uint_as_float(r.p[2]), __uint_as_float(r.p[3])};
+        l.pre1 = {__uint_as_float(r.p[4]), __uint_as_float(r.p[5]), __uint_as_float(r.p[6]), __uint_as_float(r.p[7])};
+        l.pos_range = {__uint_as_float(r.q[0]), __uint_as_float(r.q[1]), __uint_as_float(r.q[2]), __uint_as_float(r.q[3])};
+        l.cos_inner = __uint_as_float(r.inner); l.cos_outer = __uint_as_float(r.outer);
+        return l;
+    };
+    LightRaw lraw = light_issue(n_lights != 0u ? (const void*)f.lights_pre : (const void*)f.lean_tail, n_lights != 0u ? lights : (const void*)f.lean_tail, 0u);
     const float f0b = ior_to_f0(1.5f);
     sf.F0 = mix3(splat3(fminf(f0b, 1.0f)), base, sf.metallic);
     sf.f90 = mixf(1.0f, 1.0f, sf.metallic);
@@ -1801,31 +1881,23 @@
     lit.ndv_raw = ndv; lit.F0max = fmaxf(fmaxf(sf.F0.x, sf.F0.y), sf.F0.z); lit.df90max = sf.f90 - lit.F0max;
     lit.ndv_dir = sf.n_dot_v_dir; lit.ndv4 = 4.0f * sf.n_dot_v_dir; lit.a2m1 = sf.a2m1; lit.a2_g1v = sf.a2 * sf.g1_v; lit.gk = sf.gk; lit.one_m_gk = sf.one_m_gk;
     lit.occlusion = occlusion;
-    f3 color;
-    asm volatile("; MARK ibl");
     {
-        const f3 prefiltered = lean::prefiltered(sc, reflect3(-sf.v, sf.n), sf.roughness);
-        const f3 irradiance = lean::irradiance(sc, sf.n);
         const float n_dot_v = sf.n_dot_v_ibl;
         const f3 F_view = fresnel_schlick_f90(n_dot_v, sf.F0, sf.f90);
         const float F_view_max = fmaxf(fmaxf(F_view.x, F_view.y), F_view.z);
         const f3 base_layer = (base * (1.0f / kPi)) * irradiance;
         const float k_d = (1.0f - F_view_max) * (1.0f - sf.metallic);
         const f3 base_contribution = (base_layer * k_d) * occlusion;
-        const f2 lut = lean::brdf_lut(sc->lut_rg16f, sc->lut_w, sc->lut_h, n_dot_v, sf.roughness);
+        const f2 lut = lean::lut_blend(taps);
         const f3 spec_term = sf.F0 * lut.x + splat3(sf.f90 * lut.y);
         const f3 specular = (prefiltered * spec_term) * mixf(1.0f, occlusion, 0.5f);
         color = (base_contribution + specular) + emissive;
     }
-    asm volatile("; MARK lights");
-    const uint32_t n_lights = min(cload<uint32_t>(sc->buf[AWSM_BUF_LIGHTS_INFO], 0u), f.lights_cap);
-    const void* lights = sc->buf[AWSM_BUF_LIGHTS];
-    for (uint32_t i = 0; i < n_lights; i++) {
-        const f32x4 pre0 = cload<f32x4>(f.lights_pre, i * 32u), pre1 = cload<f32x4>(f.lights_pre, i * 32u + 16u);
+    auto shade_light = [&](const LightRec& L) {
+        const f32x4 pre0 = L.pre0, pre1 = L.pre1, pos_range = L.pos_range;
         const uint32_t kind = (uint32_t)pre0.w;
         f3 light_dir = {pre0.x, pre0.y, pre0.z}, radiance = {pre1.x, pre1.y, pre1.z};
         if (kind == 2u || kind == 3u) {
-            const f32x4 pos_range = cload<f32x4>(lights, i * 64u);
             const f3 stl = mk3(pos_range.x, pos_range.y, pos_range.z) - world_position;
             const float d2 = fm::fdot(stl, stl);
             const float inv_d = d2 > 0.0f ? fm::rsq(d2) : 0.0f;
@@ -1835,18 +1907,29 @@
             else { const float fo = 1.0f - fm::fdiv(dist * dist, pos_range.w * pos_range.w); att = fm::fdiv(saturate(fo * fo), dist * dist + 1.0f); }
             const f3 to_light = stl * inv_d;
             if (kind == 3u) {
-                const f32x4 dir_inner = cload<f32x4>(lights, i * 64u + 16u), kind_outer = cload<f32x4>(lights, i * 64u + 48u);
                 const float cos_l = fm::fdot(to_light, -light_dir);
-                const float sm = saturate(fm::fdiv(cos_l - kind_outer.y, dir_inner.w - kind_outer.y));
+                const float sm = saturate(fm::fdiv(cos_l - L.cos_outer, L.cos_inner - L.cos_outer));
                 att = att * (sm * sm);
             }
             light_dir = to_light;
             radiance = radiance * att;
 #ifndef AWSM_NO_LIGHT_SKIP
-            if (__builtin_amdgcn_ballot_w64(!(att == 0.0f)) == 0ull) continue;
+            if (__builtin_amdgcn_ballot_w64(!(att == 0.0f)) == 0ull) return;
 #endif
         } else if (kind != 1u) { light_dir = {0.0f, 0.0f, 0.0f}; radiance = {0.0f, 0.0f, 0.0f}; }
         lean::direct(lit, light_dir, radiance, color);
+    };
+    asm volatile("; MARK lights");
+    light_wait(lraw);
+    if (n_lights != 0u) {
+        LightRec cur = light_unpack(lraw);
+        for (uint32_t i = 1u; i < n_lights; i++) {
+            LightRaw nraw = light_issue(f.lights_pre, lights, i);
+            shade_light(cur);
+            light_wait(nraw);
+            cur = light_unpack(nraw);
+        }
+        shade_light(cur);
     }
     asm volatile("; MARK store");
     if (ITEMS) { item->color = color; return true; }
@@ -1855,8 +1938,8 @@
     return true;
 }
 template <int GRAD, bool MSAA>
-AWSM_DI void lean_block(const DevScene* __restrict__ sc, const FrameDev& f, const ShadeBlock& b, const uint32_t wg, const uint32_t tid, LeanStage* __restrict__ st) {
-    (void)lean_core<GRAD, MSAA, false>(sc, f, b, wg, tid, st, nullptr);
+AWSM_DI void lean_block(const DevScene* __restrict__ sc, const FrameDev& f, const ShadeBlock& b, const uint32_t wg, const uint32_t tid, LeanStage* __restrict__ st, const LeanGate gate) {
+    (void)lean_core<GRAD, MSAA, false>(sc, f, b, wg, tid, st, nullptr, gate);
 }
 #ifndef AWSM_ANISO_WAVES
 #define AWSM_ANISO_WAVES 4
@@ -1871,7 +1954,16 @@
 template <bool PERSIST, int GRAD, bool MSAA>
 __global__ __launch_bounds__(256) __attribute__((amdgpu_waves_per_eu(GRAD == 2 ? AWSM_ANISO_WAVES : (GRAD ? AWSM_LEAN_GRAD_WAVES : (PERSIST ? 5 : AWSM_LEAN_WAVES))))) void k_shade_lean(const DevScene* __restrict__ sc, FrameDev f) {
     __shared__ LeanStage stage[4];
-    if (frame_poisoned(f)) return;
+    LeanGate gate = {false, false, 0u};
+    constexpr bool kBatchedEntry = !PERSIST && GRAD == 0 && !MSAA;
+    if (!kBatchedEntry) { if (frame_poisoned(f)) return; }
+    else {
+        asm volatile("" :: "s"(f.width), "s"(f.sy0), "s"(f.sy1), "s"(f.tiles_y), "s"(f.tile_row0), "s"(f.band_n), "s"(f.out_compact), "s"(f.vis), "s"(f.hud_vis),
+                     "s"(f.out_rgba16f), "s"(f.out_rgba32f), "s"(f.frame_serial), "s"(f.poison), "s"(sc));
+        const uint32_t* const pz = f.poison;
+        gate.pending = true; gate.armed = pz != nullptr;
+        gate.word = SBatch<uint32_t>::issue(pz ? (const void*)pz : (const void*)f.vis, 0u);
+    }
 #ifdef AWSM_LEAN_PRIO
     __builtin_amdgcn_s_setprio(AWSM_LEAN_PRIO);
 #endif
@@ -1899,10 +1991,10 @@
             if (lane == 0u) nxt = atomicAdd(ctr0 + c * 16u, 1u);
         }
         const uint32_t kb = j >> 2, bcol = kb & ((1u << lp) - 1u), brow = (kb >> lp) * 8u + xcd;
-        if (bcol < bx_n && j < share) {
+        if ((bcol < bx_n) & (j < share)) {
             ShadeBlock b;
             shade_block_at(f, b, brow, bcol);
-            lean_block<GRAD, MSAA>(sc, f, b, ((kb >> lp) * bx_n + bcol) * 8u + xcd, ((j & 3u) << 6) | lane, st);
+            lean_block<GRAD, MSAA>(sc, f, b, ((kb >> lp) * bx_n + bcol) * 8u + xcd, ((j & 3u) << 6) | lane, st, gate);
         }
         if (!PERSIST) break;
     }
```
